# lcicek/Critic-VAE

Measured on AMD Instinct MI355X. Metric: VAE train-step images/sec on 64x64x3 frames, higher is better.
Workload: dtype f32

## Files before the change

### critic-vae_amd/csrc/api.hip

```cpp
#include "common.h"
#include "../../include/cvae.h"
#include <stdarg.h>
#include <stdio.h>
#include <stdlib.h>
#include <string.h>
#include <cmath>
#include <string>
#include <vector>

static thread_local char g_err[512] = "";
void cvae_set_error(const char* fmt, ...) {
    va_list ap;
    va_start(ap, fmt);
    vsnprintf(g_err, sizeof(g_err), fmt, ap);
    va_end(ap);
}

static constexpr int PROBE_IDS = 32, PROBE_CAP = 128;
struct ProbeSlot { hipEvent_t e0[PROBE_CAP], e1[PROBE_CAP]; int n = 0; bool made = false; };
struct ProbeState { uint32_t mask = 0; ProbeSlot slot[PROBE_IDS]; };
static thread_local ProbeSlot* g_probe_cur = nullptr;
void cvae_probe_begin(hipStream_t st) {
    ProbeSlot* p = g_probe_cur;
    if (p && p->n < PROBE_CAP) (void)hipEventRecord(p->e0[p->n], st);
}
void cvae_probe_end(hipStream_t st) {
    ProbeSlot* p = g_probe_cur;
    if (p && p->n < PROBE_CAP) { (void)hipEventRecord(p->e1[p->n], st); p->n++; }
}

int cvae_num_cus() {
    constexpr int NCACHE = 64;
    static std::atomic<int> cached[NCACHE];
    int dev = 0;
    hipError_t e = hipGetDevice(&dev);
    if (e != hipSuccess) { cvae_set_error("cvae_num_cus: hipGetDevice failed (%s); assuming 256 compute units", hipGetErrorString(e)); return 256; }
    const bool cacheable = dev >= 0 && dev < NCACHE;
    int n = cacheable ? cached[dev].load(std::memory_order_relaxed) : 0;
    if (n > 0) return n;
    e = hipDeviceGetAttribute(&n, hipDeviceAttributeMultiprocessorCount, dev);
    if (e != hipSuccess || n <= 0) {
        cvae_set_error("cvae_num_cus: compute-unit query failed on device %d (%s); assuming 256", dev, hipGetErrorString(e));
        return 256;
    }
    if (cacheable) cached[dev].store(n, std::memory_order_relaxed);
    return n;
}

int persistent_grid(int wgs_per_cu, int num_items) {
    static const int maxwg = [] { const char* e = getenv("CVAE_PERSIST_MAXWG"); const int n = e ? atoi(e) : 0; return n > 0 ? n : 0; }();
    int G = wgs_per_cu * cvae_num_cus();
    if (maxwg > 0 && G > maxwg) G = maxwg;
    G -= G % 8;
    if (G < 8) G = 8;
    return G < num_items ? G : num_items;
}
extern "C" int32_t cvae_conv_route(int32_t precision, int32_t width, int32_t layer, int32_t dgrad, int64_t batch) {
    if ((width != 64 && width != 128) || layer < 0 || layer > 3 || precision < 0 || precision > 3 || batch < 1 || batch > 0x7fffffffLL) return CVAE_EINVAL;
    if (layer == 0 && (precision != 1 || dgrad != 0)) return CVAE_EINVAL;
    return conv_route(precision, layer, width, dgrad != 0, batch).family;
}

struct ParamEntry { std::string name; int64_t offset, numel; };

struct WsLayout {
    int64_t y[4], a[4], coef[4], bnpart[4];
    int64_t zcat, h, o[4];
    int64_t dout4, d_o[4], d_h, d_zcat, d_a[4], d_y[4];
    int64_t wc[3];
    int64_t xp;
    int64_t wpack;
    int64_t ms, scratch_w, scratch, total;
};

struct cvae_handle_s {
    cvae_config cfg;
    std::vector<ParamEntry> params;
    int64_t param_total;
    int K;
    int enc_w[4], enc_b[4], enc_g[4], enc_be[4], fc_w, fc_b, dec_w[5], dec_b[5], di_w, di_b;
    hipStream_t side = nullptr;
    hipEvent_t ev_ready[8] = {}, ev_side = nullptr;
    bool streams_ready = false;
    const void* xp_ws = nullptr;
    int xp_B = 0;
    struct { int pass = 0, next = 0, B = 0; const void* ws = nullptr; const double* rec = nullptr; } sync;
    ProbeState probe;
};

struct ProbeArm {
    ProbeArm(cvae_handle_s* h, int kind, int layer) {
        const int id = kind * 9 + layer;
        g_probe_cur = (h->probe.mask >> id) & 1u ? &h->probe.slot[id] : nullptr;
    }
    ~ProbeArm() { g_probe_cur = nullptr; }
};

static int ensure_streams(cvae_handle_s* h) {
    if (h->streams_ready) return 0;
    int lo = 0, hi = 0;
    hipError_t e = hipDeviceGetStreamPriorityRange(&lo, &hi);
    if (e == hipSuccess) e = hipStreamCreateWithPriority(&h->side, hipStreamNonBlocking, lo);
    for (int i = 0; i < 8 && e == hipSuccess; ++i) e = hipEventCreateWithFlags(&h->ev_ready[i], hipEventDisableTiming);
    if (e == hipSuccess) e = hipEventCreateWithFlags(&h->ev_side, hipEventDisableTiming);
    if (e != hipSuccess) { cvae_set_error("side stream setup failed: %s", hipGetErrorString(e)); return (int)e; }
    h->streams_ready = true;
    return 0;
}

static int layer_h(const cvae_handle_s* h, int layer) { return kLayers[layer].h * (h->cfg.width / 64); }

static WsLayout carve(const cvae_handle_s* h, int B) {
    WsLayout w{};
    const int W = h->cfg.width;
    int64_t off = 0;
    auto take = [&](int64_t n) { int64_t o = off; off += align_up(n, 64); return o; };
    const bool b16 = h->cfg.precision == 1;
    auto act = [&](int64_t elems) { return take(b16 ? (elems + 1) / 2 : elems); };
    for (int l = 0; l < 4; ++l) {
        const int64_t H = layer_h(h, l), C = kLayers[l].cout;
        w.y[l] = act(B * H * H * C);
        w.a[l] = act(B * (H / 2) * (H / 2) * C);
        w.coef[l] = take(C * 4);
        w.bnpart[l] = take((int64_t)2 * bn_num_tiles(l, W, B) * C);
        w.d_y[l] = l == 0 ? -1 : act(B * H * H * C);
        w.d_a[l] = act(B * (H / 2) * (H / 2) * C);
    }
    w.zcat = take((int64_t)B * 33);
    w.d_zcat = take((int64_t)B * 33);
    w.h = act((int64_t)B * h->K);
    w.d_h = act((int64_t)B * h->K);
    for (int i = 0; i < 4; ++i) {
        const int64_t H = layer_h(h, 4 + i), C = kLayers[4 + i].cout;
        w.o[i] = act(B * H * H * C);
        w.d_o[i] = act(B * H * H * C);
    }
    w.dout4 = take(b16 ? 0 : (int64_t)B * 3 * W * W);
    for (int i = 0; i < 3; ++i) w.wc[i] = take(conv_up_wc_floats(5 + i));
    w.xp = take(b16 ? (int64_t)B * W * W * 2 : 0);
    w.wpack = take(h->cfg.precision != 0 ? conv_bf16_pack_floats(h->cfg.precision >= 2 ? 3 : 1) : 0);
    w.ms = take(msssim_ws_floats(W, B));
    int64_t sc = 0, scw = 0;
    auto mx = [&](int64_t v) { if (v > sc) sc = v; };
    for (int l = 1; l <= 4; ++l) { if (wgrad_ws_floats(l, W, B) > scw) scw = wgrad_ws_floats(l, W, B);
        if (h->cfg.precision == 1 && conv_bf16_supported(l, W) && wgrad_bf16_ws_floats(l, W, B) > scw) scw = wgrad_bf16_ws_floats(l, W, B);
        if (h->cfg.precision >= 2 && conv_bf16_supported(l, W) && wgrad_split_ws_floats(l, W, B) > scw) scw = wgrad_split_ws_floats(l, W, B);
        mx(conv_fwd_ws_floats(l, W, B)); mx(conv_dgrad_ws_floats(l, W, B)); }
    for (int l = 5; l <= 7; ++l) { if (conv_up_wgrad_ws_floats(l, W, B) > scw) scw = conv_up_wgrad_ws_floats(l, W, B); mx(conv_up_ws_floats(l, W, B)); }
    if (e1_wgrad_ws_floats(W, B) > scw) scw = e1_wgrad_ws_floats(W, B);
    w.scratch_w = take(scw);
    mx(scw + 36 * 128 * 64);
    mx(d4_bwd_ws_floats(W, B));
    for (int l = 0; l < 4; ++l) { mx(bn_bwd_ws_floats(l, W, B)); mx(bn_fwd_ws_floats(l, W)); }
    mx(fc_ws_floats(W, B));
    mx(colsum_ws_floats(0, 256));
    w.scratch = take(sc);
    w.total = off;
    return w;
}

static void add_param(cvae_handle_s* h, int* idx, const char* name, int64_t numel) {
    *idx = (int)h->params.size();
    h->params.push_back(ParamEntry{name, h->param_total, numel});
    h->param_total += align_up(numel, 64);
}

extern "C" {

const char* cvae_version(void) { return "critic-vae_amd 0.3 (gfx950; fp32 MFMA, bf16 MFMA with bf16 storage)"; }
const char* cvae_last_error(void) { return g_err; }

int cvae_create(const cvae_config* cfg, cvae_handle* out) {
    if (!cfg || !out) { cvae_set_error("cvae_create: null argument"); return CVAE_EINVAL; }
    if (cfg->width != 64 && cfg->width != 128) { cvae_set_error("cvae_create: width %d not supported (64 or 128)", cfg->width); return CVAE_EUNSUPPORTED; }
    if (cfg->precision < 0 || cfg->precision > 3) { cvae_set_error("cvae_create: precision %d not supported (0 = fp32, 1 = bf16 MFMA, 2 = fp32 emulated by 3-way bf16 splits)", cfg->precision); return CVAE_EUNSUPPORTED; }
    cvae_handle_s* h = new cvae_handle_s();
    h->cfg = *cfg;
    h->param_total = 0;
    h->K = 256 * (cfg->width / 16) * (cfg->width / 16);
    char nm[64];
    for (int l = 0; l < 4; ++l) {
        snprintf(nm, sizeof nm, "enc%d.w", l); add_param(h, &h->enc_w[l], nm, (int64_t)25 * kLayers[l].cin * kLayers[l].cout);
        snprintf(nm, sizeof nm, "enc%d.b", l); add_param(h, &h->enc_b[l], nm, kLayers[l].cout);
        snprintf(nm, sizeof nm, "enc%d.gamma", l); add_param(h, &h->enc_g[l], nm, kLayers[l].cout);
        snprintf(nm, sizeof nm, "enc%d.beta", l); add_param(h, &h->enc_be[l], nm, kLayers[l].cout);
    }
    add_param(h, &h->fc_w, "fc.w", (int64_t)h->K * 64);
    add_param(h, &h->fc_b, "fc.b", 64);
    for (int i = 0; i < 5; ++i) {
        snprintf(nm, sizeof nm, "dec%d.w", i); add_param(h, &h->dec_w[i], nm, (int64_t)25 * kLayers[4 + i].cin * kLayers[4 + i].cout);
        snprintf(nm, sizeof nm, "dec%d.b", i); add_param(h, &h->dec_b[i], nm, kLayers[4 + i].cout);
    }
    add_param(h, &h->di_w, "decin.w", (int64_t)33 * h->K);
    add_param(h, &h->di_b, "decin.b", h->K);
    *out = h;
    return CVAE_OK;
}

void cvae_destroy(cvae_handle h) {
    if (!h) return;
    if (h->streams_ready) {
        for (int i = 0; i < 8; ++i) (void)hipEventDestroy(h->ev_ready[i]);
        (void)hipEventDestroy(h->ev_side);
        (void)hipStreamDestroy(h->side);
    }
    delete h;
}

int64_t cvae_param_total(cvae_handle h) { return h->param_total; }
int32_t cvae_param_count(cvae_handle h) { return (int32_t)h->params.size(); }
const char* cvae_param_name(cvae_handle h, int32_t i) { return h->params[i].name.c_str(); }
int64_t cvae_param_offset(cvae_handle h, int32_t i) { return h->params[i].offset; }
int64_t cvae_param_numel(cvae_handle h, int32_t i) { return h->params[i].numel; }
int64_t cvae_workspace_bytes(cvae_handle h, int32_t batch) { return carve(h, batch).total * 4; }
int64_t cvae_bn_state_floats(cvae_handle) { return 2 * 480; }

int64_t cvae_ws_offset(cvae_handle h, int32_t batch, const char* name) {
    const WsLayout w = carve(h, batch);
    char nm[32];
    for (int l = 0; l < 4; ++l) {
        snprintf(nm, sizeof nm, "y%d", l); if (!strcmp(name, nm)) return w.y[l];
        snprintf(nm, sizeof nm, "a%d", l); if (!strcmp(name, nm)) return w.a[l];
        snprintf(nm, sizeof nm, "d_y%d", l); if (!strcmp(name, nm)) return w.d_y[l];
        snprintf(nm, sizeof nm, "d_a%d", l); if (!strcmp(name, nm)) return w.d_a[l];
        snprintf(nm, sizeof nm, "coef%d", l); if (!strcmp(name, nm)) return w.coef[l];
        snprintf(nm, sizeof nm, "o%d", l); if (!strcmp(name, nm)) return w.o[l];
        snprintf(nm, sizeof nm, "d_o%d", l); if (!strcmp(name, nm)) return w.d_o[l];
    }
    if (!strcmp(name, "zcat")) return w.zcat;
    if (!strcmp(name, "d_zcat")) return w.d_zcat;
    if (!strcmp(name, "h")) return w.h;
    if (!strcmp(name, "d_h")) return w.d_h;
    if (!strcmp(name, "dout4")) return w.dout4;
    if (!strcmp(name, "scratch")) return w.scratch;
    if (!strcmp(name, "ms")) return w.ms;
    if (!strcmp(name, "xp")) return h->cfg.precision == 1 ? w.xp : -1;
    return -1;
}

static const int kBnOff[4] = {0, 32, 96, 224};
static const int64_t kSyncOff[9] = {0, 97, 289, 673, 1441, 1452, 1964, 2220, 2348};
static const int64_t kSyncCnt[9] = {97, 192, 384, 768, 11, 512, 256, 128, 64};
static const int64_t kSyncCount = 96;
static_assert(2348 + 64 == CVAE_SYNC_DOUBLES, "sync record size");
int cvae_decode(cvae_handle h, int32_t B, const float* zcat, const float* params, float* recon, void* wsv, void* stream);
int cvae_backward_phases(cvae_handle h, int32_t B, const float* x, const float* pred, const float* eps, const float* params,
                         const float* logvar, const float* recon, const float* d_recon, const float* d_mu,
                         const float* d_logvar, void* wsv, float* grads, int32_t phase_mask, void* stream);

#define P_(idx) (params + h->params[(idx)].offset)
#define G_(idx) (grads + h->params[(idx)].offset)
#define RC(call) do { int rc_ = (call); if (rc_) return rc_; } while (0)

static bool use_bf16(cvae_handle h, int layer) {
    if (h->cfg.precision >= 2 && layer > 4) return false;
    return h->cfg.precision != 0 && conv_bf16_supported(layer, h->cfg.width);
}
static bool io_bf16(cvae_handle h) { return h->cfg.precision == 1; }
static bool use_bf16_wgrad(cvae_handle h, int layer) { return h->cfg.precision == 1 && conv_bf16_supported(layer, h->cfg.width); }
static bool use_split_wgrad(cvae_handle h, int layer) {
    if (h->cfg.precision < 2 || layer < 1 || layer > 4 || !conv_bf16_supported(layer, h->cfg.width)) return false;
    return conv_wgrad_split_supported(h->cfg.precision == 3 ? 6 : 9);
}
static int bf16_splits(cvae_handle h) { return h->cfg.precision >= 2 ? 3 : 1; }
static int bf16_mode(cvae_handle h) { return h->cfg.precision == 2 ? 3 : (h->cfg.precision == 3 ? 6 : 1); }
static int conv_wgrad(cvae_handle h, int layer, int B, const float* in, const float* dout, float* dw, float* dbias, float* ws, hipStream_t st) {
    const int W = h->cfg.width;
    if (use_bf16_wgrad(h, layer)) return launch_conv_wgrad_bf16(layer, W, B, in, dout, dw, dbias, ws, st);
    if (use_split_wgrad(h, layer)) return launch_conv_wgrad_split(layer, W, bf16_mode(h) == 6 ? 6 : 9, B, in, dout, dw, dbias, ws, st);
    return launch_conv_wgrad(layer, W, B, in, dout, dw, dbias, ws, st);
}
static int pack_bf16_weights(cvae_handle h, const float* params, float* ws, const WsLayout& w, hipStream_t st) {
    if (!use_bf16(h, 1)) return 0;
    const float* wl[4] = {P_(h->enc_w[1]), P_(h->enc_w[2]), P_(h->enc_w[3]), P_(h->dec_w[0])};
    return launch_pack_w_bf16(wl, ws + w.wpack, bf16_splits(h), st);
}

static int check(cvae_handle h, int32_t batch, const void* ws) {
    if (!h) { cvae_set_error("null handle"); return CVAE_EINVAL; }
    if (batch < 1 || batch > h->cfg.max_batch) { cvae_set_error("batch %d outside [1, %d]", batch, h->cfg.max_batch); return CVAE_EINVAL; }
    if (!ws) { cvae_set_error("null workspace"); return CVAE_ENOWS; }
    return 0;
}

struct FwdCtx {
    cvae_handle h; int B, W, train; const float* x; const float* params; float* bn_state; float* ws; void* wsv; WsLayout w; hipStream_t st;
    int tpp = 1;
    float* xp() const { return train && conv_route(1, 0, W, false, B).family == E1_PACKED_FRAME ? ws + w.xp : nullptr; }
    bool two_pass(int l) const { return l == 0 && h->cfg.precision == 1; }
    int conv(int l) {
        tpp = 1;
        if (two_pass(l)) {
            if (train) RC(launch_e1_fwd(W, B, x, P_(h->enc_w[0]), P_(h->enc_b[0]), nullptr, ws + w.bnpart[0], st, true, 1, nullptr, nullptr, xp()));
            h->xp_ws = xp() ? wsv : nullptr; h->xp_B = B;
            return 0;
        }
        if (l == 0) { ProbeArm pa(h, 0, 0); RC(launch_e1_fwd(W, B, x, P_(h->enc_w[0]), P_(h->enc_b[0]), ws + w.y[0], ws + w.bnpart[0], st)); }
        else if (use_bf16(h, l)) { ProbeArm pa(h, 0, l); RC(launch_conv_fwd_bf16(l, W, bf16_mode(h), B, ws + w.a[l - 1], ws + w.wpack, P_(h->enc_b[l]), ws + w.y[l], ws + w.bnpart[l], ws + w.scratch, st, &tpp)); }
        else { ProbeArm pa(h, 0, l); RC(launch_conv_fwd(l, W, B, ws + w.a[l - 1], P_(h->enc_w[l]), P_(h->enc_b[l]), ws + w.y[l], ws + w.bnpart[l], ws + w.scratch, st)); }
        return 0;
    }
    int stats(int l, double* sync) {
        if (sync) return launch_bn_fwd_record(l, W, B, ws + w.bnpart[l], ws + w.scratch, st, tpp, sync + kSyncOff[l], l == 0 ? sync + kSyncCount : nullptr);
        return launch_bn_fwd_finalize(l, W, B, ws + w.bnpart[l], P_(h->enc_g[l]), P_(h->enc_be[l]), bn_state + kBnOff[l],
                                      bn_state + 480 + kBnOff[l], ws + w.coef[l], ws + w.scratch, train, st, tpp);
    }
    int finish(int l, const double* sync) {
        return launch_bn_fwd_finish(l, W, sync + kSyncOff[l], sync + kSyncCount, P_(h->enc_g[l]), P_(h->enc_be[l]), bn_state + kBnOff[l],
                                    bn_state + 480 + kBnOff[l], ws + w.coef[l], st);
    }
    int apply(int l) {
        if (two_pass(l)) {
            ProbeArm pa(h, 0, 0);
            return launch_e1_fwd(W, B, x, P_(h->enc_w[0]), P_(h->enc_b[0]), ws + w.y[0], nullptr, st, true, 2, ws + w.coef[0], ws + w.a[0],
                                 xp());
        }
        return launch_bn_pool_act_fwd(l, W, B, ws + w.y[l], ws + w.coef[l], ws + w.a[l], st, io_bf16(h));
    }
};

int cvae_forward(cvae_handle h, int32_t B, const float* x, const float* pred, const float* eps, const float* params,
                 float* bn_state, float* mu, float* logvar, float* recon, void* wsv, int32_t train, void* stream) {
    RC(check(h, B, wsv));
    hipStream_t st = (hipStream_t)stream;
    float* ws = (float*)wsv;
    const WsLayout w = carve(h, B);
    const int W = h->cfg.width;
    RC(pack_bf16_weights(h, params, ws, w, st));
    FwdCtx f{h, B, W, train, x, params, bn_state, ws, wsv, w, st};
    for (int l = 0; l < 4; ++l) {
        RC(f.conv(l));
        RC(f.stats(l, nullptr));
        RC(f.apply(l));
    }
    RC(launch_fc_fwd(W, B, ws + w.a[3], P_(h->fc_w), P_(h->fc_b), eps, pred, mu, logvar, ws + w.zcat, ws + w.scratch, st, io_bf16(h)));
    if (!recon) return 0;
    return cvae_decode(h, B, nullptr, params, recon, wsv, stream);
}

int cvae_decode(cvae_handle h, int32_t B, const float* zcat, const float* params, float* recon, void* wsv, void* stream) {
    RC(check(h, B, wsv));
    hipStream_t st = (hipStream_t)stream;
    float* ws = (float*)wsv;
    const WsLayout w = carve(h, B);
    const int W = h->cfg.width;
    if (zcat) {
        hipError_t e = hipMemcpyAsync(ws + w.zcat, zcat, (size_t)B * 33 * sizeof(float), hipMemcpyDeviceToDevice, st);
        if (e != hipSuccess) { cvae_set_error("cvae_decode: copy failed: %s", hipGetErrorString(e)); return (int)e; }
        RC(pack_bf16_weights(h, params, ws, w, st));
    }
    RC(launch_decin_fwd(W, B, ws + w.zcat, P_(h->di_w), P_(h->di_b), ws + w.h, st, io_bf16(h)));
    {
        const float* wsrc[3] = {P_(h->dec_w[1]), P_(h->dec_w[2]), P_(h->dec_w[3])};
        float* wdst[3] = {ws + w.wc[0], ws + w.wc[1], ws + w.wc[2]};
        RC(launch_collapse_w3(wsrc, wdst, st));
    }
    if (use_bf16(h, 5)) {
        const float* wcs[3] = {ws + w.wc[0], ws + w.wc[1], ws + w.wc[2]};
        RC(launch_pack_up_bf16(wcs, ws + w.wpack, bf16_splits(h), st));
    }
    for (int i = 0; i < 4; ++i) {
        ProbeArm pa(h, 0, 4 + i);
        if (i == 0) {
// ... 980 lines not shown
```

### critic-vae_amd/csrc/common.h

```cpp
#pragma once
#include <hip/hip_runtime.h>
#include <stdint.h>
#include <stddef.h>
#include <atomic>

typedef float f32x16 __attribute__((ext_vector_type(16)));
typedef float f32x4 __attribute__((ext_vector_type(4)));
typedef __bf16 bf16x8 __attribute__((ext_vector_type(8)));

typedef __bf16 bf16x4 __attribute__((ext_vector_type(4)));

template <typename AT> struct Act;
template <> struct Act<float> {
    static constexpr bool BF16 = false;
    static __device__ __forceinline__ float ld(const float* p, size_t i) { return p[i]; }
    static __device__ __forceinline__ void st(float* p, size_t i, float v) { p[i] = v; }
    static __device__ __forceinline__ f32x4 ld4(const float* p, size_t i) { return *reinterpret_cast<const f32x4*>(p + i); }
    static __device__ __forceinline__ void st4(float* p, size_t i, f32x4 v) { *reinterpret_cast<f32x4*>(p + i) = v; }
    template <int V> using Vec = float __attribute__((ext_vector_type(V)));
    template <int V> static __device__ __forceinline__ Vec<V> ldv(const float* p, size_t i) {
        static_assert(V == 1 || V == 4, "fp32 storage: scalar or float4 accesses");
        return *reinterpret_cast<const Vec<V>*>(p + i);
    }
    template <int V> static __device__ __forceinline__ void stv(float* p, size_t i, Vec<V> v) {
        static_assert(V == 1 || V == 4, "fp32 storage: scalar or float4 accesses");
        *reinterpret_cast<Vec<V>*>(p + i) = v;
    }
};
template <> struct Act<__bf16> {
    static constexpr bool BF16 = true;
    static __device__ __forceinline__ float ld(const float* p, size_t i) { return (float)reinterpret_cast<const __bf16*>(p)[i]; }
    static __device__ __forceinline__ void st(float* p, size_t i, float v) { reinterpret_cast<__bf16*>(p)[i] = (__bf16)v; }
    static __device__ __forceinline__ f32x4 ld4(const float* p, size_t i) {
        const bf16x4 v = *reinterpret_cast<const bf16x4*>(reinterpret_cast<const __bf16*>(p) + i);
        return f32x4{(float)v[0], (float)v[1], (float)v[2], (float)v[3]};
    }
    static __device__ __forceinline__ void st4(float* p, size_t i, f32x4 v) {
        bf16x4 o;
        o[0] = (__bf16)v[0]; o[1] = (__bf16)v[1]; o[2] = (__bf16)v[2]; o[3] = (__bf16)v[3];
        *reinterpret_cast<bf16x4*>(reinterpret_cast<__bf16*>(p) + i) = o;
    }
    static __device__ __forceinline__ bf16x4 ld4raw(const float* p, size_t i) { return *reinterpret_cast<const bf16x4*>(reinterpret_cast<const __bf16*>(p) + i); }
    static __device__ __forceinline__ bf16x8 ld8(const float* p, size_t i) { return *reinterpret_cast<const bf16x8*>(reinterpret_cast<const __bf16*>(p) + i); }
    static __device__ __forceinline__ void st8(float* p, size_t i, bf16x8 v) { *reinterpret_cast<bf16x8*>(reinterpret_cast<__bf16*>(p) + i) = v; }
    template <int V> using Vec = __bf16 __attribute__((ext_vector_type(V)));
    template <int V> static __device__ __forceinline__ Vec<V> ldv(const float* p, size_t i) {
        static_assert(V == 8, "bf16 storage: 16-byte units of 8 elements");
        return ld8(p, i);
    }
    template <int V> static __device__ __forceinline__ void stv(float* p, size_t i, Vec<V> v) {
        static_assert(V == 8, "bf16 storage: 16-byte units of 8 elements");
        st8(p, i, v);
    }
};

typedef short short4v __attribute__((ext_vector_type(4)));
typedef short short8v __attribute__((ext_vector_type(8)));
__device__ __forceinline__ bf16x8 tr_frag(const __bf16* p0, const __bf16* p1) {
    const short4v lo = __builtin_amdgcn_ds_read_tr16_b64_v4i16((__attribute__((address_space(3))) short4v*)p0);
    const short4v hi = __builtin_amdgcn_ds_read_tr16_b64_v4i16((__attribute__((address_space(3))) short4v*)p1);
    const short8v v = __builtin_shufflevector(lo, hi, 0, 1, 2, 3, 4, 5, 6, 7);
    return __builtin_bit_cast(bf16x8, v);
}

#define CVAE_LATENT 32
#define CVAE_ZCAT 33

struct LayerDesc { int cin, cout, h, up; };
static constexpr LayerDesc kLayers[9] = {
    {3, 32, 64, 0}, {32, 64, 32, 0}, {64, 128, 16, 0}, {128, 256, 8, 0},
    {256, 128, 4, 0}, {128, 64, 8, 1}, {64, 32, 16, 1}, {32, 32, 32, 1}, {32, 3, 64, 1}};

struct TileGeom { int TW, TH, IMGS, PX_PER_IMG, TILES_PER_IMG; };
__host__ __device__ constexpr TileGeom tile_geom(int H) {
    const int TW = H < 32 ? H : 32;
    const int TH = (128 / TW) < H ? (128 / TW) : H;
    return TileGeom{TW, TH, 128 / (TW * TH), TW * TH, (H / TW) * (H / TH)};
}
template <int H>
struct Tile {
    static constexpr int TW = tile_geom(H).TW, TH = tile_geom(H).TH;
    static constexpr int IMGS = tile_geom(H).IMGS;
    static constexpr int HTW = TW + 4, HTH = TH + 4;
    static constexpr int HPI = HTW * HTH;
    static constexpr int HP = IMGS * HPI;
    static constexpr int PS = ((HP + 5) / 8) * 8 + 2;
    static constexpr int TILES_X = H / TW, TILES_Y = H / TH;
    static constexpr int TILES_PER_IMG = tile_geom(H).TILES_PER_IMG;
    static_assert(TW * TH * IMGS == 128, "tile must hold 128 pixels");
};

__host__ __device__ inline int cdiv(int a, int b) { return (a + b - 1) / b; }

__device__ __forceinline__ void vm_drained() { __builtin_amdgcn_s_waitcnt(0x0F70); }

__device__ __forceinline__ int xcd_tile(int x, int G) { return (G & 7) ? x : (x & 7) * (G >> 3) + (x >> 3); }
inline int64_t align_up(int64_t v, int64_t a) { return (v + a - 1) / a * a; }

__device__ __forceinline__ float wave_sum(float v) {
#pragma unroll
    for (int o = 32; o > 0; o >>= 1) v += __shfl_xor(v, o, 64);
    return v;
}
__device__ __forceinline__ double wave_sum_d(double v) {
#pragma unroll
    for (int o = 32; o > 0; o >>= 1) v += __shfl_xor(v, o, 64);
    return v;
}

__device__ __forceinline__ bool wg_arrive_last(unsigned* counter, unsigned total, unsigned* lds_word) {
    asm volatile("s_waitcnt vmcnt(0)" ::: "memory");
    __syncthreads();
    if (threadIdx.x == 0) {
        __builtin_amdgcn_fence(__ATOMIC_RELEASE, "agent");
        asm volatile("s_waitcnt vmcnt(0)" ::: "memory");
        const unsigned t = __hip_atomic_fetch_add(counter, 1u, __ATOMIC_RELAXED, __HIP_MEMORY_SCOPE_AGENT);
        const bool last = t == total - 1;
        if (last) {
            __hip_atomic_store(counter, 0u, __ATOMIC_RELAXED, __HIP_MEMORY_SCOPE_AGENT);
            __builtin_amdgcn_fence(__ATOMIC_ACQUIRE, "agent");
            asm volatile("s_waitcnt vmcnt(0)" ::: "memory");
        }
        *lds_word = last ? 1u : 0u;
    }
    __syncthreads();
    return *lds_word != 0u;
}

void cvae_probe_begin(hipStream_t st);
void cvae_probe_end(hipStream_t st);

void cvae_set_error(const char* fmt, ...);
#define CVAE_CHECK_LAUNCH()                                                        \
    do {                                                                           \
        hipError_t e_ = hipGetLastError();                                         \
        if (e_ != hipSuccess) {                                                    \
            cvae_set_error("%s:%d launch failed: %s", __FILE__, __LINE__,          \
                           hipGetErrorString(e_));                                 \
            return (int)e_;                                                        \
        }                                                                          \
    } while (0)

struct DeviceOnce { std::atomic<uint64_t> mask{0}; };
inline int cvae_grant_lds(DeviceOnce& once, const void* kernel, int bytes) {
    int dev = 0;
    hipError_t e = hipGetDevice(&dev);
    const uint64_t bit = 1ull << (dev & 63);
    if (e == hipSuccess && (once.mask.load(std::memory_order_acquire) & bit)) return 0;
    if (e == hipSuccess) e = hipFuncSetAttribute(kernel, hipFuncAttributeMaxDynamicSharedMemorySize, bytes);
    if (e != hipSuccess) { cvae_set_error("dynamic LDS opt-in (%d bytes) failed: %s", bytes, hipGetErrorString(e)); return (int)e; }
    once.mask.fetch_or(bit, std::memory_order_release);
    return 0;
}

int cvae_num_cus();
int persistent_grid(int wgs_per_cu, int num_items);

enum ConvFamily { CONV_PER_TILE = 0, CONV_PS = 1, CONV_BIG = 2, E1_PACKED_FRAME = 1 };
struct ConvRoute {
    ConvFamily family;
    int tilesPerPartial;
};
ConvRoute conv_route(int precision, int layer, int width, bool dgrad, int64_t B);

int launch_conv_fwd(int layer, int width, int B, const float* in, const float* w, const float* bias,
                    float* out, float* bnpart, float* ws, hipStream_t st);
int64_t conv_fwd_ws_floats(int layer, int width, int B);
int launch_conv_dgrad(int layer, int width, int B, const float* dout, const float* w,
                      const float* mask_src, float* din, float* ws, hipStream_t st);
int64_t conv_dgrad_ws_floats(int layer, int width, int B);
bool conv_bf16_supported(int layer, int width);
int64_t conv_bf16_pack_floats(int ns);
int launch_pack_w_bf16(const float* const w[4], float* packed, int ns, hipStream_t st);
int launch_conv_fwd_bf16(int layer, int width, int ns, int B, const float* in, const float* packed, const float* bias, float* out,
                         float* bnpart, float* ws, hipStream_t st, int* tilesPerPartial = nullptr);
int launch_conv_dgrad_bf16(int layer, int width, int ns, int B, const float* dout, const float* packed, float* din, float* ws, hipStream_t st);
int launch_pack_up_bf16(const float* const wc[3], float* packed, int ns, hipStream_t st);
int launch_conv_up_fwd_bf16(int layer, int width, int ns, int B, const float* in, const float* packed, const float* bias, float* out, hipStream_t st);
int launch_conv_up_dgrad_bf16(int layer, int width, int ns, int B, const float* dout, const float* packed, const float* aux, float* din, hipStream_t st);
int64_t wgrad_bf16_ws_floats(int layer, int width, int B);
int launch_conv_wgrad_bf16(int layer, int width, int B, const float* in, const float* dout, float* dw, float* dbias, float* ws, hipStream_t st);
bool conv_wgrad_split_supported(int products);
int64_t wgrad_split_ws_floats(int layer, int width, int B);
int launch_conv_wgrad_split(int layer, int width, int products, int B, const float* in, const float* dout, float* dw, float* dbias,
                            float* ws, hipStream_t st);
int launch_splitk_bias_relu(const float* slab, const float* bias, float* out, int64_t slice, int KS, int C, hipStream_t st, bool out_bf16 = false);
int64_t wgrad_ws_floats(int layer, int width, int B);
int launch_conv_wgrad(int layer, int width, int B, const float* in, const float* dout, float* dw,
                      float* dbias, float* ws, hipStream_t st);
int launch_reduce_slabs(const float* slab, float* dst, int64_t n, int S, int64_t stride, hipStream_t st,
                        float* mid = nullptr, bool out_bf16 = false);
int launch_colsum(const float* src, int64_t rows, int C, float* dst, float* ws, hipStream_t st);
int64_t colsum_ws_floats(int64_t rows, int C);
static constexpr int CS_BLOCKS = 128;
__device__ __forceinline__ void colsum_stage1_block(const float* __restrict__ src, int64_t rows, int C, float* __restrict__ part,
                                                    int blk, int nblk, float* red) {
    const int c = threadIdx.x % C, rl = threadIdx.x / C, RL = 256 / C;
    const int64_t per = (rows + nblk - 1) / nblk;
    const int64_t r0 = blk * per;
    int64_t r1 = r0 + per; if (r1 > rows) r1 = rows;
    float acc = 0.f;
    for (int64_t r = r0 + rl; r < r1; r += RL) acc += src[r * C + c];
    red[threadIdx.x] = acc;
    __syncthreads();
    if (rl == 0) {
        for (int k = 1; k < RL; ++k) acc += red[k * C + c];
        part[(size_t)blk * C + c] = acc;
    }
}
int64_t col_reduce_ws_floats(int W);
int launch_col_reduce_partial(const float* in, int R, int W, int64_t stride, float* ws, hipStream_t st,
                              const float** rows_out, int* R_out, int64_t* stride_out);
int launch_col_reduce(const float* in, int R, int W, int64_t stride, float* out, float* ws, hipStream_t st, int skip_col0 = -1);
int launch_e1_fwd(int width, int B, const float* x, const float* w, const float* bias, float* y,
                  float* bnpart, hipStream_t st, bool bf16 = false, int pass = 0, const float* coef = nullptr, float* a1 = nullptr,
                  float* xp = nullptr);
int launch_e1_wgrad(int width, int B, const float* x, const float* dy, float* dw, float* dbias, float* ws,
                    hipStream_t st, bool bf16 = false, const float* const* fuse = nullptr,
                    const float* xp = nullptr);
const float* bn_bwd_bcoef(int layer, int width, int B, const float* ws);
int64_t e1_wgrad_ws_floats(int width, int B);
int launch_d4_fwd(int width, int B, const float* in, const float* w, const float* bias, float* recon,
                  hipStream_t st, bool bf16io = false);
int64_t d4_bwd_ws_floats(int width, int B);
int launch_d4_bwd(int width, int B, const float* o3, const float* d_recon, const float* recon,
                  const float* w, float* dout, float* d_o3, float* dw, float* db, float* ws,
                  hipStream_t st, bool bf16io = false);
int64_t conv_up_wc_floats(int layer);
int launch_collapse_w(int layer, const float* w, float* wc, hipStream_t st);
int launch_collapse_w3(const float* const w[3], float* const wc[3], hipStream_t st);
int64_t conv_up_ws_floats(int layer, int width, int B);
int launch_conv_up_fwd(int layer, int width, int B, const float* in, const float* wc, const float* bias,
                       float* out, float* ws, hipStream_t st);
int launch_conv_up_dgrad(int layer, int width, int B, const float* dout, const float* wc, const float* aux,
                         float* din, float* ws, hipStream_t st);
int64_t conv_up_wgrad_ws_floats(int layer, int width, int B);
int launch_conv_up_wgrad(int layer, int width, int B, const float* in, const float* dout, float* dw,
                         float* dbias, float* ws, hipStream_t st, bool bf16 = false);
int launch_up_wgrad_bf16_main(int layer, int width, int B, const float* in, const float* dout, float* slab, int Smax, int* S_out, hipStream_t st,
                              int* plan = nullptr);
int conv_wgrad_bf16_plan(int layer, int width, int B, int plan[3]);
int conv_up_wgrad_bf16_plan(int layer, int width, int B, int plan[3]);
int bn_num_tiles(int layer, int width, int B);
int launch_bn_fwd_finalize(int layer, int width, int B, const float* bnpart, const float* gamma,
                           const float* beta, float* run_mean, float* run_var, float* coef,
                           float* ws, int train, hipStream_t st, int tilesPerPartial = 1);
int launch_bn_fwd_record(int layer, int width, int B, const float* bnpart, float* ws, hipStream_t st, int tilesPerPartial,
                         double* rec, double* count);
int launch_bn_fwd_finish(int layer, int width, const double* rec, const double* count, const float* gamma, const float* beta,
                         float* run_mean, float* run_var, float* coef, hipStream_t st);
int64_t bn_fwd_ws_floats(int layer, int width);
int launch_bn_pool_act_fwd(int layer, int width, int B, const float* y, const float* coef, float* a,
                           hipStream_t st, bool bf16io = false);
int64_t bn_bwd_ws_floats(int layer, int width, int B);
int launch_bn_pool_act_bwd(int layer, int width, int B, const float* y, const float* a,
                           const float* da, const float* coef, const float* gamma, float* dy,
                           float* dgamma, float* dbeta, float* dbias, float* ws, hipStream_t st, bool bf16io = false,
                           int stage = 0, double* rec = nullptr, const double* count = nullptr);
struct LatentPlan {
    int fc_fwd_gemm;
    int di_imgs, di_blocks;
    int db_bgemm, db_gemm;
    int df_imgs, fb_bgemm, fb_dflat, fb_colsum;
    int fb_split;
};
LatentPlan latent_plan(int width, int B, int num_cus);
int64_t fc_ws_floats(int width, int B);
int launch_fc_fwd(int width, int B, const float* flat, const float* wfc, const float* bfc,
                  const float* eps, const float* pred, float* mu, float* logvar, float* zcat,
                  float* ws, hipStream_t st, bool bf16io = false);
int launch_decin_fwd(int width, int B, const float* zcat, const float* wd, const float* bd, float* h,
                     hipStream_t st, bool bf16io = false);
int launch_decin_bwd(int width, int B, const float* zcat, const float* dh, const float* wd, float* dwd,
                     float* dbd, float* dzcat, float* ws, hipStream_t st, bool bf16io = false);
int launch_fc_bwd(int width, int B, const float* flat, const float* wfc, const float* dzcat,
                  const float* eps, const float* logvar, const float* dmu_loss,
                  const float* dlv_loss, float* dwfc, float* dbfc, float* dflat, float* ws,
                  hipStream_t st, bool bf16io = false);
struct LossObjective { float w_ms, w_mse, kw; int used; };
constexpr int MSSSIM_SLAB_DOUBLES = 32 * 11;
int launch_objective_pixels(int width, int B, const float* recon, const float* x, const float* const* F, const float* coef,
                            float* dx, const float* mu, const float* logvar, float* d_mu, float* d_logvar,
                            LossObjective obj, double* slab, unsigned* ticket, float* scalars, hipStream_t st);
int64_t msssim_ws_floats(int width, int B);
int launch_msssim(int width, int B, const float* img1, const float* img2, const float* mu,
                  const float* logvar, float* ws, float* scalars, float* d_img1, float* d_mu,
                  float* d_logvar, hipStream_t st,
                  int stage = 0, double* rec = nullptr, const double* images = nullptr,
                  const LossObjective* obj = nullptr);
void msssim_score_slots(int width, int B, int64_t part[5], int64_t* scratch);
int launch_msssim_finish_rec(int width, const double* rec, const double* images, float* scalars, float* coef, hipStream_t st);
int64_t score_state_bytes();
int launch_score_init(void* state, hipStream_t st);
int launch_score(int width, int B, const float* x, const float* mu, const float* logvar, const float* recon, float* ms,
                 float* per_image, void* state, hipStream_t st);
int launch_score_finish(int width, void* state, float* scalars, hipStream_t st);
namespace critic_layout {
constexpr int CW1 = 0, CB1 = 216, CW2 = 224, CB2 = 800, CW3 = 808, CB3 = 1384, CW4 = 1392, CB4 = 2544,
              CW5 = 2560, CB5 = 10752, CF1W = 10784, CF1B = 11808, CF2W = 11840, CF2B = 11872;
constexpr int CRITIC_PARAMS = 11873;
}
int critic_param_count();
int launch_critic_fwd(int width, int B, const float* x, const float* critic_params, float* pred, hipStream_t st);
int launch_preprocess_u8(int width, int B, const uint8_t* u8, float* x, hipStream_t st);
int critic_train_floats();
int64_t critic_grad_scratch_bytes(int B);
int launch_critic_grad(int width, int B, const float* x, const float* target, const uint8_t* keep, float scale, int loss_kind,
                       const float* critic_params, float* grads, float* pred, float* loss_scalars, uint8_t* decisions,
                       void* scratch, hipStream_t st);
int64_t critic_score_state_bytes();
int64_t critic_score_scratch_bytes(int B);
int launch_critic_score_init(void* state, hipStream_t st);
int launch_critic_score(int B, const uint8_t* frames, const float* targets, int64_t n, const int64_t* idx, const float* critic_params,
                        float* rows, void* state, hipStream_t st);
int launch_critic_collect(int B, const float* x, const float* critic_params, float* pred, float* const e[5], hipStream_t st);
int launch_critic_saliency(int B, const float* x, const float* critic_params, int steps, float* pred, float* grad, float* map,
                           float* max_values, uint8_t* decisions, hipStream_t st);
int launch_critic_occlusion(int B, const float* x, const float* critic_params, int patch, float fill_r, float fill_g, float fill_b,
                            float* pred, float* drop, float* map, float* max_values, hipStream_t st);
int launch_curate_select(int n_traj, const int64_t* off, int64_t n_frames, const float* preds, int collect,
                         int64_t total_images, int64_t* running, int64_t* counts, int64_t* first, int64_t* span,
                         int64_t* sel, hipStream_t st);
int launch_gather_frames_u8(int width, const uint8_t* src, const float* src_pred, int64_t n_src, const int64_t* sel,
                            int64_t max_count, const int64_t* span, uint8_t* dst, float* dst_pred, int64_t capacity,
                            hipStream_t st);
int launch_preprocess_u8_gather(int width, int B, const uint8_t* frames, const float* preds, int64_t n, const int64_t* idx,
                                float* x, float* pred, hipStream_t st);
int launch_curate_select_recon(int n_traj, const int64_t* off, int64_t n_frames, const float* preds, int collect,
                               int64_t total_images, int64_t* running, int64_t* counts, int64_t* first, int64_t* sel_first,
                               int64_t* span, int64_t* ent_frame, int32_t* ent_kind, int64_t* ent_sel, int64_t* sel,
                               hipStream_t st);
int launch_recon_zcat(int n_entries, const int64_t* ent_sel, const int32_t* ent_kind, const float* mu, const float* sel_pred,
                      int64_t n_sel, float* zcat, hipStream_t st);
int launch_inject_zcat(int n_images, int n_rewards, const float* mu, const float* rewards, float* zcat, hipStream_t st);
int launch_gather_f32(int width, int B, const float* frames, const float* preds, int64_t n, const int64_t* idx, float* x,
                      float* pred, hipStream_t st);
int launch_preprocess_u8_gather_aug(int width, int B, const uint8_t* frames, const float* preds, int64_t n, const int64_t* idx,
                                    const struct cvae_augment& aug, float* x, float* pred, int32_t* applied, hipStream_t st);
int launch_gather_f32_aug(int width, int B, const float* frames, const float* preds, int64_t n, const int64_t* idx,
                          const struct cvae_augment& aug, float* x, float* pred, int32_t* applied, hipStream_t st);
int launch_diff_grey(int width, int B, const float* a, const float* b, float* diff, hipStream_t st);
int64_t crf_scratch_bytes(int width, int B);
int launch_dense_crf(int width, int B, const uint8_t* frames, const float* prob1, const struct cvae_crf_params& p,
                     uint8_t* labels, float* q1, void* scratch, hipStream_t st);
int launch_diff_normalize(int width, int B, const float* diff, double mean_max, double factor, int thr, const uint8_t* gt,
                          uint8_t* u8, uint8_t* mask, int64_t* counts, int64_t* hist, hipStream_t st);
int launch_mask_counts(int width, int B, const uint8_t* mask, const uint8_t* gt, int64_t* counts, hipStream_t st);
int launch_compose_frames(int width, int B, int n_panels, const struct cvae_panel* panels, int ih, int clamp, const uint8_t* overlay,
                          const uint8_t* atlas, int n_labels, int lh, int lw, const int32_t* label_idx, int lx, int ly,
                          uint8_t* out, hipStream_t st);
int launch_grads_bf16(const float* src_f32, void* bf16_buf, float* dst_f32, int64_t n, hipStream_t st);
int launch_adam(float* p, const float* g, float* m, float* v, int64_t n, int step, float lr, float b1,
                float b2, float eps, float gscale, hipStream_t st);
int64_t guard_state_bytes();
int launch_guard_init(void* state, int64_t applied, int64_t skipped, hipStream_t st);
int launch_grad_stats(const float* g, int64_t n, float gscale, float max_norm, int skip_nonfinite, float lr, float b1, float b2,
                      void* state, hipStream_t st);
int launch_adam_guarded(float* p, const float* g, float* m, float* v, int64_t n, float eps, const void* state, hipStream_t st);
struct cvae_opt_args;
int launch_adam_opt(float* p, const float* g, float* m, float* v, int64_t n, int step, float lr, float b1, float b2, float eps,
                    float gscale, const cvae_opt_args* opt, float* ema, const float* aux, float* aux_ema, int32_t n_aux, hipStream_t st);
int launch_adam_guarded_opt(float* p, const float* g, float* m, float* v, int64_t n, float eps, const void* state,
                            const cvae_opt_args* opt, float* ema, const float* aux, float* aux_ema, int32_t n_aux, hipStream_t st);
struct cvae_tensor_stat;
int launch_trace_push(void* ring, int64_t capacity, int64_t step, float lr, const float* scalars, int n_scalars,
                      const void* guard_state, hipStream_t st);
int launch_tensor_stats(const float* p, const float* g, const float* m, const float* v, int64_t n, int32_t n_tensors,
                        const int64_t* begin, const int64_t* end, int64_t step, float lr, float b1, float b2, float eps, float gscale,
                        const void* guard_state, cvae_tensor_stat* out, void* scratch, hipStream_t st);
int64_t tensor_stats_scratch_bytes(int32_t n_tensors, const int64_t* begin, const int64_t* end);
int tensor_stats_plan(int32_t n_tensors, const int64_t* begin, const int64_t* end, int32_t* chunk, int32_t* items, int32_t* grid);
int launch_zero(float* p, int64_t n, hipStream_t st);
struct PadGaps { int64_t off[32]; int len[32]; int n; };
int launch_zero_gaps(float* grads, const PadGaps& gaps, hipStream_t st);
struct Scale3 { const float* g; const float* src[3]; float* dst[3]; int64_t n[3]; };
int launch_scale3(const Scale3& a, hipStream_t st);
```

### critic-vae_amd/csrc/conv_mfma.hip

```cpp
#include "common.h"
#include "conv_epilogue.h"


struct ConvRouteRow { int precision, layer, width; bool dgrad; ConvFamily family; int tilesPerPartial; };
static constexpr ConvRouteRow kConvRoutes[] = {
    {0, 1, 64, false, CONV_PS, 1}, {0, 2, 64, false, CONV_PS, 1}, {0, 3, 64, false, CONV_PS, 1},
    {0, 2, 64, true, CONV_PS, 1}, {0, 3, 64, true, CONV_PS, 1},
    {0, 1, 128, false, CONV_PS, 1}, {0, 2, 128, false, CONV_PS, 1}, {0, 2, 128, true, CONV_PS, 1},
    {1, 1, 64, false, CONV_BIG, 8}, {1, 2, 64, false, CONV_BIG, 4}, {1, 3, 64, false, CONV_BIG, 4},
    {1, 1, 64, true, CONV_BIG, 1}, {1, 2, 64, true, CONV_BIG, 1}, {1, 3, 64, true, CONV_BIG, 1},
    {1, 1, 128, false, CONV_BIG, 8}, {1, 2, 128, false, CONV_BIG, 4}, {1, 3, 128, false, CONV_BIG, 4},
    {1, 1, 128, true, CONV_BIG, 1}, {1, 2, 128, true, CONV_BIG, 1}, {1, 3, 128, true, CONV_BIG, 1},
    {1, 4, 128, false, CONV_PS, 1},
    {1, 0, 64, false, E1_PACKED_FRAME, 1}, {1, 0, 128, false, E1_PACKED_FRAME, 1},
};

ConvRoute conv_route(int precision, int layer, int width, bool dgrad, int64_t B) {
    static const bool per_tile_only = [] { const char* e = getenv("CVAE_CONV_PER_TILE"); return e && e[0] == '1'; }();
    const ConvRoute per_tile{CONV_PER_TILE, 1};
    for (const ConvRouteRow& r : kConvRoutes) {
        if (r.precision != precision || r.layer != layer || r.width != width || r.dgrad != dgrad) continue;
        if (layer == 0) {
            if (B * width * width * 8 + (2 * width + 2) * 8 >= (1ll << 31)) return per_tile;
            return {r.family, r.tilesPerPartial};
        }
        if (per_tile_only) return per_tile;
        const int64_t h = kLayers[layer].h * width / 64, c = kLayers[layer].cin > kLayers[layer].cout ? kLayers[layer].cin : kLayers[layer].cout;
        if (B * h * h * c * (precision == 1 ? 2 : 4) >= (1ll << 31)) return per_tile;
        return {r.family, r.tilesPerPartial};
    }
    return per_tile;
}


struct ConvArgs {
    const float* in;
    const float* w;
    const float* bias;
    const float* aux;
    float* out;
    float* bnpart;
    int B;
    int64_t sliceFloats;
};

template <int NT> struct KChunk { static constexpr int KC = NT == 32 ? 32 : 16, KCP = KC + 1; };


template <int KCH, int NCH, int H, bool DGRAD, int NT, int EPI, int KSPLIT>
__global__ __launch_bounds__(256) void conv5x5_mfma_kernel(ConvArgs a) {
    using T = Tile<H>;
    constexpr int NB = NT / 32;
    constexpr int KC = KChunk<NT>::KC, KCP = KChunk<NT>::KCP, QPP = KC / 4;
    constexpr int IN_FLOATS = KC * T::PS;
    constexpr int W_FLOATS = DGRAD ? 5 * NT * KCP : 5 * KC * NT;
    constexpr int EPI_FLOATS = (EPI == EPI_POOLSUM_MASK) ? 128 * (NT + 1) : 4 * 32 * 36;
    constexpr int SMEM = (IN_FLOATS + W_FLOATS) > EPI_FLOATS ? (IN_FLOATS + W_FLOATS) : EPI_FLOATS;
    __shared__ __attribute__((aligned(16))) float smem[SMEM];
    float* lds_in = smem;
    float* lds_w = smem + IN_FLOATS;

    const int tid = threadIdx.x, lane = tid & 63, wave = tid >> 6;
    const int li = lane & 31, lh = lane >> 5;
    const int mt = xcd_tile(blockIdx.x, gridDim.x), n0 = blockIdx.y * NT;
    const int tileInImg = mt % T::TILES_PER_IMG;
    const int img0 = (mt / T::TILES_PER_IMG) * T::IMGS;
    const int ty0 = (tileInImg / T::TILES_X) * T::TH, tx0 = (tileInImg % T::TILES_X) * T::TW;

    const int m = wave * 32 + li;
    const int pimg = m / (T::TH * T::TW), prem = m % (T::TH * T::TW);
    const int aBase = lh * T::PS + pimg * T::HPI + (prem / T::TW) * T::HTW + (prem % T::TW);
    const int bBase = DGRAD ? (li * KCP + lh) : (lh * NT + li);

    f32x16 acc[NB];
#pragma unroll
    for (int nb = 0; nb < NB; ++nb)
#pragma unroll
        for (int v = 0; v < 16; ++v) acc[nb][v] = 0.f;

    constexpr int WQ = 5 * KC * NT / 4;
    constexpr int WPT = (WQ + 255) / 256;
    f32x4 wreg[WPT];

    auto load_w = [&](int st) {
        const int cc = st / 5, r = st % 5;
#pragma unroll
        for (int i = 0; i < WPT; ++i) {
            const int q = tid + i * 256;
            if (WQ % 256 == 0 || q < WQ) {
                const float* src;
                if (!DGRAD) {
                    const int row = q / (NT / 4), c4 = q % (NT / 4);
                    const int s = row / KC, kc = row % KC;
                    src = a.w + (size_t)((r * 5 + s) * KCH + cc * KC + kc) * NCH + n0 + c4 * 4;
                } else {
                    const int c4 = q % QPP, rown = q / QPP;
                    const int n = rown % NT, s = rown / NT;
                    src = a.w + (size_t)((24 - (r * 5 + s)) * NCH + n0 + n) * KCH + cc * KC + c4 * 4;
                }
                wreg[i] = *reinterpret_cast<const f32x4*>(src);
            }
        }
    };
    auto store_w = [&]() {
#pragma unroll
        for (int i = 0; i < WPT; ++i) {
            const int q = tid + i * 256;
            if (WQ % 256 == 0 || q < WQ) {
                if (!DGRAD) {
                    *reinterpret_cast<f32x4*>(lds_w + q * 4) = wreg[i];
                } else {
                    const int c4 = q % QPP, rown = q / QPP;
                    float* d = lds_w + rown * KCP + c4 * 4;
                    d[0] = wreg[i].x; d[1] = wreg[i].y; d[2] = wreg[i].z; d[3] = wreg[i].w;
                }
            }
        }
    };
    constexpr int NQ = T::HP * (KC / 4), IPT = (NQ + 255) / 256;
    f32x4 ireg[IPT];
    auto load_input = [&](int cc) {
#pragma unroll
        for (int i = 0; i < IPT; ++i) {
            const int q = tid + i * 256;
            const int c4 = q % QPP, hp = q / QPP;
            const int img = hp / T::HPI, rem = hp - img * T::HPI;
            const int hy = rem / T::HTW, hx = rem - hy * T::HTW;
            const int gy = ty0 + hy - 2, gx = tx0 + hx - 2, ib = img0 + img;
            f32x4 v = {0.f, 0.f, 0.f, 0.f};
            if ((NQ % 256 == 0 || q < NQ) && (unsigned)gy < (unsigned)H && (unsigned)gx < (unsigned)H && ib < a.B)
                v = *reinterpret_cast<const f32x4*>(a.in + ((size_t)(ib * H + gy) * H + gx) * KCH + cc * KC + c4 * 4);
            ireg[i] = v;
        }
    };
    auto store_input = [&]() {
#pragma unroll
        for (int i = 0; i < IPT; ++i) {
            const int q = tid + i * 256;
            if (NQ % 256 == 0 || q < NQ) {
                float* d = lds_in + ((q % QPP) * 4) * T::PS + (q / QPP);
                d[0] = ireg[i].x; d[T::PS] = ireg[i].y; d[2 * T::PS] = ireg[i].z; d[3 * T::PS] = ireg[i].w;
            }
        }
    };

    static_assert((KCH / KC) % KSPLIT == 0, "split-K must divide the channel chunks");
    constexpr int NST = (KCH / KC) / KSPLIT * 5;
    const int st0 = blockIdx.z * NST, st1 = st0 + NST;
    [[maybe_unused]] float biasv[NB];
    if constexpr (KSPLIT == 1 && (EPI == EPI_BIAS_BNSTAT || EPI == EPI_BIAS_RELU)) load_bias<NT, EPI>(biasv, a.bias, n0);
    load_w(st0);
    load_input(st0 / 5);
    for (int st = st0; st < st1; ++st) {
        const int r = st % 5;
        __syncthreads();
        if (r == 0) store_input();
        store_w();
        if (r == 0 && st + 5 < st1) load_input(st / 5 + 1);
        if (st + 1 < st1) load_w(st + 1);
        __syncthreads();
        const float* ap = lds_in + aBase + r * T::HTW;
        __builtin_amdgcn_iglp_opt(0);
#pragma unroll
        for (int s = 0; s < 5; ++s) {
#pragma unroll
            for (int j = 0; j < KC / 2; ++j) {
                const float av = ap[(2 * j) * T::PS + s];
#pragma unroll
                for (int nb = 0; nb < NB; ++nb) {
                    const float bv = DGRAD ? lds_w[bBase + (s * NT + nb * 32) * KCP + 2 * j]
                                           : lds_w[bBase + (s * KC + 2 * j) * NT + nb * 32];
                    acc[nb] = __builtin_amdgcn_mfma_f32_32x32x2f32(av, bv, acc[nb], 0, 0, 0);
                }
            }
        }
    }
    vm_drained();

    if (KSPLIT > 1) {
        epilogue_store<H, NT, NCH, EPI_PLAIN>(acc, a.out + (size_t)blockIdx.z * a.sliceFloats, nullptr, smem, a.B,
                                              mt, n0, img0, ty0, tx0);
    } else if (EPI == EPI_BIAS_BNSTAT || EPI == EPI_BIAS_RELU || EPI == EPI_PLAIN) {
        apply_bias<NT, EPI>(acc, biasv);
        __builtin_amdgcn_sched_barrier(0);
        epilogue_store<H, NT, NCH, EPI>(acc, a.out, a.bnpart, smem, a.B, mt, n0, img0, ty0, tx0);
    } else {
        __syncthreads();
        float* lo = smem;
#pragma unroll
        for (int nb = 0; nb < NB; ++nb)
#pragma unroll
            for (int v = 0; v < 16; ++v) {
                const int mm = wave * 32 + (v & 3) + 8 * (v >> 2) + 4 * lh;
                lo[mm * (NT + 1) + nb * 32 + li] = acc[nb][v];
            }
        __syncthreads();
        constexpr int PTW = T::TW / 2, PTH = T::TH / 2, HO = H / 2;
        for (int q = tid; q < 32 * NT; q += 256) {
            const int c = q % NT, pp = q / NT;
            const int im = pp / (PTW * PTH), rem = pp % (PTW * PTH);
            const int py = rem / PTW, px = rem % PTW, ib = img0 + im;
            if (ib >= a.B) continue;
            const int m00 = im * T::TH * T::TW + (2 * py) * T::TW + 2 * px;
            const float sum = (lo[m00 * (NT + 1) + c] + lo[(m00 + 1) * (NT + 1) + c]) +
                              (lo[(m00 + T::TW) * (NT + 1) + c] + lo[(m00 + T::TW + 1) * (NT + 1) + c]);
            const size_t o = ((size_t)(ib * HO + ty0 / 2 + py) * HO + tx0 / 2 + px) * NCH + n0 + c;
            a.out[o] = a.aux[o] > 0.f ? sum : 0.f;
        }
    }
}

template <int KCH, int NCH, int H, bool DGRAD, int NT, int EPI, int KSPLIT = 1>
static int run(const ConvArgs& a, hipStream_t st) {
    using T = Tile<H>;
    static_assert(KCH % KChunk<NT>::KC == 0 && NCH % NT == 0, "channel tiling");
    dim3 grid(cdiv(a.B, T::IMGS) * T::TILES_PER_IMG, NCH / NT, KSPLIT);
    cvae_probe_begin(st);
    hipLaunchKernelGGL((conv5x5_mfma_kernel<KCH, NCH, H, DGRAD, NT, EPI, KSPLIT>), grid, dim3(256), 0, st, a);
    cvae_probe_end(st);
    CVAE_CHECK_LAUNCH();
    return 0;
}

template <int KCH, int NCH, bool DGRAD, int NT, int KSPLIT>
__global__ __launch_bounds__(256) void conv4x4_row_kernel(ConvArgs a) {
    constexpr int NB = NT / 32;
    constexpr int KC = KChunk<NT>::KC, KCP = KChunk<NT>::KCP, QPP = KC / 4;
    constexpr int PXS = 33, PS = 16 * PXS + 2;
    constexpr int IN_FLOATS = KC * PS;
    constexpr int W_FLOATS = DGRAD ? 5 * NT * KCP : 5 * KC * NT;
    __shared__ __attribute__((aligned(16))) float smem[IN_FLOATS + W_FLOATS];
    float* lds_in = smem;
    float* lds_w = smem + IN_FLOATS;
    static_assert(IN_FLOATS % 4 == 0, "weight slab stays 16-byte aligned");
    const int tid = threadIdx.x, lane = tid & 63, wave = tid >> 6, li = lane & 31, lh = lane >> 5;
    const int ya = (blockIdx.x & 1) * 2, img0 = (blockIdx.x >> 1) * 32, n0 = blockIdx.y * NT;
    const int r0 = ya == 0 ? 1 : 0, r1 = ya == 0 ? 4 : 3;
    const int aBase = lh * PS + li;
    const int bBase = DGRAD ? (li * KCP + lh) : (lh * NT + li);

    f32x16 acc[2][NB];
#pragma unroll
    for (int t = 0; t < 2; ++t)
#pragma unroll
        for (int nb = 0; nb < NB; ++nb)
#pragma unroll
            for (int v = 0; v < 16; ++v) acc[t][nb][v] = 0.f;

    constexpr int WQ = 5 * KC * NT / 4, WPT = (WQ + 255) / 256;
    f32x4 wreg[WPT];
    auto load_w = [&](int cc, int r) {
#pragma unroll
        for (int i = 0; i < WPT; ++i) {
            const int q = tid + i * 256;
            if (WQ % 256 == 0 || q < WQ) {
                const float* src;
                if (!DGRAD) {
                    const int row = q / (NT / 4), c4 = q % (NT / 4);
                    const int s = row / KC, kc = row % KC;
                    src = a.w + (size_t)((r * 5 + s) * KCH + cc * KC + kc) * NCH + n0 + c4 * 4;
                } else {
                    const int c4 = q % QPP, rown = q / QPP;
                    const int n = rown % NT, s = rown / NT;
                    src = a.w + (size_t)((24 - (r * 5 + s)) * NCH + n0 + n) * KCH + cc * KC + c4 * 4;
                }
                wreg[i] = *reinterpret_cast<const f32x4*>(src);
            }
        }
    };
    auto store_w = [&]() {
#pragma unroll
        for (int i = 0; i < WPT; ++i) {
            const int q = tid + i * 256;
            if (WQ % 256 == 0 || q < WQ) {
                if (!DGRAD) {
                    *reinterpret_cast<f32x4*>(lds_w + q * 4) = wreg[i];
                } else {
                    const int c4 = q % QPP, rown = q / QPP;
                    float* d = lds_w + rown * KCP + c4 * 4;
                    d[0] = wreg[i].x; d[1] = wreg[i].y; d[2] = wreg[i].z; d[3] = wreg[i].w;
                }
            }
        }
    };
    constexpr int NQ = 512 * QPP, IPT = NQ / 256;
    f32x4 ireg[IPT];
    auto load_input = [&](int cc) {
#pragma unroll
        for (int i = 0; i < IPT; ++i) {
            const int q = tid + i * 256, c4 = q % QPP, hp = q / QPP, ib = img0 + (hp >> 4);
            f32x4 v = {0.f, 0.f, 0.f, 0.f};
            if (ib < a.B) v = *reinterpret_cast<const f32x4*>(a.in + ((size_t)ib * 16 + (hp & 15)) * KCH + cc * KC + c4 * 4);
            ireg[i] = v;
        }
    };
    auto store_input = [&]() {
#pragma unroll
        for (int i = 0; i < IPT; ++i) {
            const int q = tid + i * 256, c4 = q % QPP, hp = q / QPP;
            float* d = lds_in + (c4 * 4) * PS + (hp & 15) * PXS + (hp >> 4);
            d[0] = ireg[i].x; d[PS] = ireg[i].y; d[2 * PS] = ireg[i].z; d[3 * PS] = ireg[i].w;
        }
    };

    static_assert((KCH / KC) % KSPLIT == 0, "split-K must divide the channel chunks");
    constexpr int CPS = (KCH / KC) / KSPLIT;
    const int c0 = blockIdx.z * CPS, c1 = c0 + CPS;
    load_w(c0, r0);
    load_input(c0);
    for (int cc = c0; cc < c1; ++cc)
        for (int r = r0; r <= r1; ++r) {
            __syncthreads();
            if (r == r0) store_input();
            store_w();
            if (r == r0 && cc + 1 < c1) load_input(cc + 1);
            if (r < r1) load_w(cc, r + 1);
            else if (cc + 1 < c1) load_w(cc + 1, r0);
            __syncthreads();
#pragma unroll
            for (int t = 0; t < 2; ++t) {
                const int yi = ya + t + r - 2;
                if ((unsigned)yi > 3u) continue;
                const int xc = wave ^ t;
                const int s0 = xc < 2 ? 2 - xc : 0, s1 = xc > 1 ? 5 - xc : 4;
                const float* ap = lds_in + aBase + (yi * 4 + xc - 2) * PXS;
                for (int s = s0; s <= s1; ++s) {
                    const float* as = ap + s * PXS;
                    const float* bs = lds_w + bBase + (DGRAD ? s * NT * KCP : s * KC * NT);
#pragma unroll
                    for (int j = 0; j < KC / 2; ++j) {
                        const float av = as[(2 * j) * PS];
#pragma unroll
                        for (int nb = 0; nb < NB; ++nb) {
                            const float bv = DGRAD ? bs[nb * 32 * KCP + 2 * j] : bs[(2 * j) * NT + nb * 32];
                            acc[t][nb] = __builtin_amdgcn_mfma_f32_32x32x2f32(av, bv, acc[t][nb], 0, 0, 0);
                        }
                    }
                }
            }
        }
    vm_drained();
    float* out = a.out + (size_t)blockIdx.z * a.sliceFloats;
#pragma unroll
    for (int t = 0; t < 2; ++t)
#pragma unroll
        for (int nb = 0; nb < NB; ++nb)
#pragma unroll
            for (int v = 0; v < 16; ++v) {
                const int ib = img0 + (v & 3) + 8 * (v >> 2) + 4 * lh;
                if (ib < a.B) out[((size_t)ib * 16 + (ya + t) * 4 + (wave ^ t)) * NCH + n0 + nb * 32 + li] = acc[t][nb][v];
            }
}

template <int KCH, int NCH, bool DGRAD, int NT, int KSPLIT>
static int run4x4(const ConvArgs& a, hipStream_t st) {
    static_assert(KCH % KChunk<NT>::KC == 0 && NCH % NT == 0, "channel tiling");
    cvae_probe_begin(st);
    hipLaunchKernelGGL((conv4x4_row_kernel<KCH, NCH, DGRAD, NT, KSPLIT>), dim3(cdiv(a.B, 32) * 2, NCH / NT, KSPLIT), dim3(256), 0, st, a);
    cvae_probe_end(st);
    CVAE_CHECK_LAUNCH();
    return 0;
}

template <typename AT>
__global__ __launch_bounds__(256) void splitk_bias_relu_kernel(const float* __restrict__ slab, const float* __restrict__ bias,
                                                               float* __restrict__ out, int64_t n4, int64_t slice, int KS, int C) {
    const int64_t i = (int64_t)blockIdx.x * 256 + threadIdx.x;
    if (i >= n4) return;
    float4 acc = *reinterpret_cast<const float4*>(bias + (i * 4) % C);
    for (int z = 0; z < KS; ++z) {
        const float4 v = *reinterpret_cast<const float4*>(slab + (size_t)z * slice + i * 4);
        acc.x += v.x; acc.y += v.y; acc.z += v.z; acc.w += v.w;
    }
    acc.x = fmaxf(acc.x, 0.f); acc.y = fmaxf(acc.y, 0.f); acc.z = fmaxf(acc.z, 0.f); acc.w = fmaxf(acc.w, 0.f);
    Act<AT>::st4(out, (size_t)i * 4, f32x4{acc.x, acc.y, acc.z, acc.w});
}

int launch_splitk_bias_relu(const float* slab, const float* bias, float* out, int64_t slice, int KS, int C, hipStream_t st, bool out_bf16) {
    if (out_bf16) hipLaunchKernelGGL(splitk_bias_relu_kernel<__bf16>, dim3((unsigned)((slice / 4 + 255) / 256)), dim3(256), 0, st, slab, bias, out,
                                     slice / 4, slice, KS, C);
    else hipLaunchKernelGGL(splitk_bias_relu_kernel<float>, dim3((unsigned)((slice / 4 + 255) / 256)), dim3(256), 0, st, slab, bias, out,
                       slice / 4, slice, KS, C);
    CVAE_CHECK_LAUNCH();
    return 0;
}

static constexpr int D0_KSPLIT = 8;
int64_t conv_fwd_ws_floats(int layer, int width, int B) {
    if (layer != 4 || width != 64) return 0;
    const int64_t h = kLayers[4].h * (width / 64);
    return (int64_t)D0_KSPLIT * B * h * h * kLayers[4].cout;
}

int launch_conv_mfma_ps(int layer, int width, bool dgrad, int B, const float* in, const float* w, const float* bias, float* out, float* bnpart, hipStream_t st);

int launch_conv_fwd(int layer, int width, int B, const float* in, const float* w, const float* bias,
                    float* out, float* bnpart, float* ws, hipStream_t st) {
    if (conv_route(0, layer, width, false, B).family == CONV_PS) return launch_conv_mfma_ps(layer, width, false, B, in, w, bias, out, bnpart, st);
    ConvArgs a{in, w, bias, nullptr, out, bnpart, B, 0};
    if (width == 64) {
        switch (layer) {
            case 1: return run<32, 64, 32, false, 64, EPI_BIAS_BNSTAT>(a, st);
            case 2: return run<64, 128, 16, false, 64, EPI_BIAS_BNSTAT>(a, st);
            case 3: return run<128, 256, 8, false, 32, EPI_BIAS_BNSTAT>(a, st);
            case 4: {
                const int64_t slice = (int64_t)B * 4 * 4 * 128;
                a.out = ws; a.sliceFloats = slice;
                int rc = run4x4<256, 128, false, 64, D0_KSPLIT>(a, st);
                if (rc) return rc;
                hipLaunchKernelGGL(splitk_bias_relu_kernel<float>, dim3((unsigned)((slice / 4 + 255) / 256)), dim3(256), 0, st,
                                   ws, bias, out, slice / 4, slice, D0_KSPLIT, 128);
                CVAE_CHECK_LAUNCH();
                return 0;
            }
        }
    }
    if (width == 128) {
        switch (layer) {
            case 1: return run<32, 64, 64, false, 64, EPI_BIAS_BNSTAT>(a, st);
            case 2: return run<64, 128, 32, false, 64, EPI_BIAS_BNSTAT>(a, st);
            case 3: return run<128, 256, 16, false, 64, EPI_BIAS_BNSTAT>(a, st);
            case 4: return run<256, 128, 8, false, 64, EPI_BIAS_RELU>(a, st);
        }
    }
    cvae_set_error("conv_fwd: unsupported layer %d at width %d", layer, width);
    return -2;
}

static constexpr int D0_DGRAD_KSPLIT = 4;
int64_t conv_dgrad_ws_floats(int layer, int width, int B) {
    if (layer != 4 || width != 64) return 0;
    return (int64_t)D0_DGRAD_KSPLIT * B * 16 * kLayers[4].cin;
}

int launch_conv_dgrad(int layer, int width, int B, const float* dout, const float* w,
                      const float* mask_src, float* din, float* ws, hipStream_t st) {
    if (!mask_src && conv_route(0, layer, width, true, B).family == CONV_PS) return launch_conv_mfma_ps(layer, width, true, B, dout, w, nullptr, din, nullptr, st);
    ConvArgs a{dout, w, nullptr, mask_src, din, nullptr, B, 0};
    if (width == 64 && layer == 4 && ws != nullptr) {
        const int64_t slice = (int64_t)B * 16 * 256;
        a.out = ws; a.sliceFloats = slice;
        int rc = run4x4<128, 256, true, 64, D0_DGRAD_KSPLIT>(a, st);
        if (rc) return rc;
        return launch_reduce_slabs(ws, din, slice, D0_DGRAD_KSPLIT, slice, st, nullptr);
    }
    if (width == 64) {
        switch (layer) {
            case 1: return run<64, 32, 32, true, 32, EPI_PLAIN>(a, st);
            case 2: return run<128, 64, 16, true, 64, EPI_PLAIN>(a, st);
            case 3: return run<256, 128, 8, true, 32, EPI_PLAIN>(a, st);
            case 4: return run<128, 256, 4, true, 32, EPI_PLAIN>(a, st);
        }
    }
    if (width == 128) {
        switch (layer) {
            case 1: return run<64, 32, 64, true, 32, EPI_PLAIN>(a, st);
            case 2: return run<128, 64, 32, true, 64, EPI_PLAIN>(a, st);
            case 3: return run<256, 128, 16, true, 64, EPI_PLAIN>(a, st);
            case 4: return run<128, 256, 8, true, 64, EPI_PLAIN>(a, st);
        }
    }
    cvae_set_error("conv_dgrad: unsupported layer %d at width %d", layer, width);
    return -2;
}
```

### critic-vae_amd/csrc/conv_up.hip

```cpp
#include "common.h"

static constexpr int KC = 16, KCP = 17;

template <int HS>
struct UpTile {
    static constexpr int TW = HS < 32 ? HS : 32;
    static constexpr int TH = (128 / TW) < HS ? (128 / TW) : HS;
    static constexpr int IMGS = 128 / (TW * TH);
    static constexpr int HTW = TW + 2, HTH = TH + 2, HPI = HTW * HTH, HP = IMGS * HPI;
    static constexpr int PS = ((HP + 5) / 8) * 8 + 2;
    static constexpr int TILES_X = HS / TW, TILES_Y = HS / TH, TILES_PER_IMG = TILES_X * TILES_Y;
};

__device__ __forceinline__ int phase_lo(int ph, int a) { return ph == 0 ? (a == 0 ? 0 : a == 1 ? 2 : 4) : (a == 0 ? 0 : a == 1 ? 1 : 3); }
__device__ __forceinline__ int phase_hi(int ph, int a) { return ph == 0 ? (a == 0 ? 1 : a == 1 ? 3 : 4) : (a == 0 ? 0 : a == 1 ? 2 : 4); }
__device__ __forceinline__ int phase_of(int ph, int r) { return ph == 0 ? (r >> 1) : ((r + 1) >> 1); }

struct CollapseJobs { const float* w[3]; float* wc[3]; int n[3]; };
__global__ __launch_bounds__(256) void collapse_w_kernel(CollapseJobs jobs) {
    const float* __restrict__ w = jobs.w[blockIdx.z];
    float* __restrict__ wc = jobs.wc[blockIdx.z];
    const int n = jobs.n[blockIdx.z];
    const int i = blockIdx.x * 256 + threadIdx.x;
    if (i >= n) return;
    const int t = blockIdx.y, p = t / 9, a = (t % 9) / 3, b = t % 3, py = p >> 1, px = p & 1;
    float acc = 0.f;
    for (int r = phase_lo(py, a); r <= phase_hi(py, a); ++r)
        for (int s = phase_lo(px, b); s <= phase_hi(px, b); ++s) acc += w[(size_t)(r * 5 + s) * n + i];
    wc[(size_t)t * n + i] = acc;
}

__global__ __launch_bounds__(256) void expand_dw_kernel(const float* __restrict__ rows, int R, int64_t stride,
                                                        float* __restrict__ dw, int n, float* __restrict__ dbias,
                                                        int cout) {
    const int i = blockIdx.x * 256 + threadIdx.x;
    if (dbias != nullptr && blockIdx.x == 0 && blockIdx.y == 0 && (int)threadIdx.x < cout) {
        float b = 0.f;
        for (int q = 0; q < R; ++q) b += rows[(size_t)q * stride + (size_t)36 * n + threadIdx.x];
        dbias[threadIdx.x] = b;
    }
    if (i >= n) return;
    const int r = blockIdx.y / 5, s = blockIdx.y % 5;
    float acc = 0.f;
#pragma unroll
    for (int p = 0; p < 4; ++p) {
        const float* src = rows + (size_t)(p * 9 + phase_of(p >> 1, r) * 3 + phase_of(p & 1, s)) * n + i;
        float a = 0.f;
        for (int q = 0; q < R; ++q) a += src[(size_t)q * stride];
        acc += a;
    }
    dw[(size_t)blockIdx.y * n + i] = acc;
}

struct UpArgs {
    const float* in;
    const float* wc;
    const float* bias;
    const float* aux;
    float* out;
    int B;
    int64_t sliceFloats;
};

template <int CIN, int COUT, int HS, int KSPLIT>
__global__ __launch_bounds__(256) void conv_up_fwd_kernel(UpArgs a) {
    using T = UpTile<HS>;
    constexpr int NT = 32, H = 2 * HS;
    constexpr int IN_FLOATS = KC * T::PS, W_FLOATS = 12 * KC * NT;
    __shared__ __attribute__((aligned(16))) float smem[IN_FLOATS + W_FLOATS];
    float* lds_in = smem;
    float* lds_w = smem + IN_FLOATS;
    const int tid = threadIdx.x, lane = tid & 63, wave = tid >> 6, li = lane & 31, lh = lane >> 5;
    const int mt = xcd_tile(blockIdx.x, gridDim.x), n0 = blockIdx.y * NT;
    const int tileInImg = mt % T::TILES_PER_IMG, img0 = (mt / T::TILES_PER_IMG) * T::IMGS;
    const int ty0 = (tileInImg / T::TILES_X) * T::TH, tx0 = (tileInImg % T::TILES_X) * T::TW;
    const int m = wave * 32 + li;
    const int pimg = m / (T::TH * T::TW), prem = m % (T::TH * T::TW);
    const int aBase = lh * T::PS + pimg * T::HPI + (prem / T::TW) * T::HTW + (prem % T::TW);
    const int bBase = lh * NT + li;

    f32x16 acc[4];
#pragma unroll
    for (int p = 0; p < 4; ++p)
#pragma unroll
        for (int v = 0; v < 16; ++v) acc[p][v] = 0.f;

    constexpr int WQ = 12 * KC * NT / 4, WPT = WQ / 256;
    f32x4 wreg[WPT];
    auto load_w = [&](int st) {
        const int cc = st / 3, ar = st % 3;
#pragma unroll
        for (int i = 0; i < WPT; ++i) {
            const int q = tid + i * 256;
            const int row = q / (NT / 4), c4 = q % (NT / 4);
            const int pb = row / KC, kc = row % KC, p = pb / 3, b = pb % 3;
            wreg[i] = *reinterpret_cast<const f32x4*>(
                a.wc + ((size_t)(p * 9 + ar * 3 + b) * CIN + cc * KC + kc) * COUT + n0 + c4 * 4);
        }
    };
    auto store_w = [&]() {
#pragma unroll
        for (int i = 0; i < WPT; ++i) *reinterpret_cast<f32x4*>(lds_w + (tid + i * 256) * 4) = wreg[i];
    };
    constexpr int NQ = T::HP * (KC / 4), IPT = (NQ + 255) / 256;
    f32x4 ireg[IPT];
    auto load_input = [&](int cc) {
#pragma unroll
        for (int i = 0; i < IPT; ++i) {
            const int q = tid + i * 256;
            const int c4 = q & 3, hp = q >> 2;
            const int img = hp / T::HPI, rem = hp - img * T::HPI;
            const int gy = ty0 + rem / T::HTW - 1, gx = tx0 + rem % T::HTW - 1, ib = img0 + img;
            f32x4 v = {0.f, 0.f, 0.f, 0.f};
            if ((NQ % 256 == 0 || q < NQ) && (unsigned)gy < (unsigned)HS && (unsigned)gx < (unsigned)HS && ib < a.B)
                v = *reinterpret_cast<const f32x4*>(a.in + ((size_t)(ib * HS + gy) * HS + gx) * CIN + cc * KC + c4 * 4);
            ireg[i] = v;
        }
    };
    auto store_input = [&]() {
#pragma unroll
        for (int i = 0; i < IPT; ++i) {
            const int q = tid + i * 256;
            if (NQ % 256 == 0 || q < NQ) {
                float* d = lds_in + ((q & 3) * 4) * T::PS + (q >> 2);
                d[0] = ireg[i].x; d[T::PS] = ireg[i].y; d[2 * T::PS] = ireg[i].z; d[3 * T::PS] = ireg[i].w;
            }
        }
    };

    static_assert((CIN / KC) % KSPLIT == 0, "split-K must divide the channel chunks");
    constexpr int NST = (CIN / KC) / KSPLIT * 3;
    const int st0 = blockIdx.z * NST, st1 = st0 + NST;
    const float bv = KSPLIT > 1 ? 0.f : a.bias[n0 + li];
    load_w(st0);
    load_input(st0 / 3);
    for (int st = st0; st < st1; ++st) {
        const int ar = st % 3;
        __syncthreads();
        if (ar == 0) store_input();
        store_w();
        if (ar == 0 && st + 3 < st1) load_input(st / 3 + 1);
        if (st + 1 < st1) load_w(st + 1);
        __syncthreads();
        const float* ap = lds_in + aBase + ar * T::HTW;
        __builtin_amdgcn_iglp_opt(0);
#pragma unroll
        for (int b = 0; b < 3; ++b)
#pragma unroll
            for (int j = 0; j < KC / 2; ++j) {
                const float av = ap[(2 * j) * T::PS + b];
#pragma unroll
                for (int p = 0; p < 4; ++p)
                    acc[p] = __builtin_amdgcn_mfma_f32_32x32x2f32(av, lds_w[bBase + ((p * 3 + b) * KC + 2 * j) * NT], acc[p], 0, 0, 0);
            }
    }
    vm_drained();
    float* out = KSPLIT > 1 ? a.out + (size_t)blockIdx.z * a.sliceFloats : a.out;
#pragma unroll
    for (int p = 0; p < 4; ++p)
#pragma unroll
        for (int v = 0; v < 16; ++v) {
            const int mm = wave * 32 + (v & 3) + 8 * (v >> 2) + 4 * lh;
            const int im = mm / (T::TH * T::TW), rem = mm % (T::TH * T::TW);
            const int oy = 2 * (ty0 + rem / T::TW) + (p >> 1), ox = 2 * (tx0 + rem % T::TW) + (p & 1), ib = img0 + im;
            float x = acc[p][v] + bv;
            if (KSPLIT == 1) x = fmaxf(x, 0.f);
            if (ib < a.B) out[((size_t)(ib * H + oy) * H + ox) * COUT + n0 + li] = x;
        }
}

template <int CIN, int COUT, int HS, int NT, int KSPLIT>
__global__ __launch_bounds__(256) void conv_up_dgrad_kernel(UpArgs a) {
    using T = UpTile<HS>;
    constexpr int NB = NT / 32, H = 2 * HS;
    constexpr int IN_FLOATS = KC * T::PS, W_FLOATS = 9 * NT * KCP;
    __shared__ __attribute__((aligned(16))) float smem[IN_FLOATS + W_FLOATS];
    float* lds_in = smem;
    float* lds_w = smem + IN_FLOATS;
    const int tid = threadIdx.x, lane = tid & 63, wave = tid >> 6, li = lane & 31, lh = lane >> 5;
    const int mt = xcd_tile(blockIdx.x, gridDim.x), n0 = blockIdx.y * NT;
    const int tileInImg = mt % T::TILES_PER_IMG, img0 = (mt / T::TILES_PER_IMG) * T::IMGS;
    const int ty0 = (tileInImg / T::TILES_X) * T::TH, tx0 = (tileInImg % T::TILES_X) * T::TW;
    const int m = wave * 32 + li;
    const int pimg = m / (T::TH * T::TW), prem = m % (T::TH * T::TW);
    const int aBase = lh * T::PS + pimg * T::HPI + (prem / T::TW + 2) * T::HTW + (prem % T::TW) + 2;
    const int bBase = li * KCP + lh;

    f32x16 acc[NB];
#pragma unroll
    for (int nb = 0; nb < NB; ++nb)
#pragma unroll
        for (int v = 0; v < 16; ++v) acc[nb][v] = 0.f;

    constexpr int WQ = 9 * NT * KC / 4, WPT = (WQ + 255) / 256;
    f32x4 wreg[WPT];
    auto load_w = [&](int st) {
        const int cc = st / 4, p = st % 4;
#pragma unroll
        for (int i = 0; i < WPT; ++i) {
            const int q = tid + i * 256;
            if (WQ % 256 == 0 || q < WQ) {
                const int c4 = q & 3, rown = q >> 2, n = rown % NT, t = rown / NT;
                wreg[i] = *reinterpret_cast<const f32x4*>(
                    a.wc + ((size_t)(p * 9 + t) * CIN + n0 + n) * COUT + cc * KC + c4 * 4);
            }
        }
    };
    auto store_w = [&]() {
#pragma unroll
        for (int i = 0; i < WPT; ++i) {
            const int q = tid + i * 256;
            if (WQ % 256 == 0 || q < WQ) {
                float* d = lds_w + (q >> 2) * KCP + (q & 3) * 4;
                d[0] = wreg[i].x; d[1] = wreg[i].y; d[2] = wreg[i].z; d[3] = wreg[i].w;
            }
        }
    };
    constexpr int NQ = T::HP * (KC / 4), IPT = (NQ + 255) / 256;
    f32x4 ireg[IPT];
    auto load_input = [&](int st) {
        const int cc = st / 4, py = (st % 4) >> 1, px = st & 1;
#pragma unroll
        for (int i = 0; i < IPT; ++i) {
            const int q = tid + i * 256;
            const int c4 = q & 3, hp = q >> 2;
            const int img = hp / T::HPI, rem = hp - img * T::HPI;
            const int yy = ty0 + rem / T::HTW - 1, xx = tx0 + rem % T::HTW - 1, ib = img0 + img;
            f32x4 v = {0.f, 0.f, 0.f, 0.f};
            if ((NQ % 256 == 0 || q < NQ) && (unsigned)yy < (unsigned)HS && (unsigned)xx < (unsigned)HS && ib < a.B)
                v = *reinterpret_cast<const f32x4*>(
                    a.in + ((size_t)(ib * H + 2 * yy + py) * H + 2 * xx + px) * COUT + cc * KC + c4 * 4);
            ireg[i] = v;
        }
    };
    auto store_input = [&]() {
#pragma unroll
        for (int i = 0; i < IPT; ++i) {
            const int q = tid + i * 256;
            if (NQ % 256 == 0 || q < NQ) {
                float* d = lds_in + ((q & 3) * 4) * T::PS + (q >> 2);
                d[0] = ireg[i].x; d[T::PS] = ireg[i].y; d[2 * T::PS] = ireg[i].z; d[3 * T::PS] = ireg[i].w;
            }
        }
    };

    static_assert((COUT / KC) % KSPLIT == 0, "split-K must divide the channel chunks");
    constexpr int NST = (COUT / KC) / KSPLIT * 4;
    const int st0 = blockIdx.z * NST, st1 = st0 + NST;
    load_w(st0);
    load_input(st0);
    for (int st = st0; st < st1; ++st) {
        __syncthreads();
        store_input();
        store_w();
        if (st + 1 < st1) { load_input(st + 1); load_w(st + 1); }
        __syncthreads();
        __builtin_amdgcn_iglp_opt(0);
#pragma unroll
        for (int t = 0; t < 9; ++t)
#pragma unroll
            for (int j = 0; j < KC / 2; ++j) {
                const float av = lds_in[aBase + (2 * j) * T::PS - (t / 3) * T::HTW - (t % 3)];
#pragma unroll
                for (int nb = 0; nb < NB; ++nb)
                    acc[nb] = __builtin_amdgcn_mfma_f32_32x32x2f32(av, lds_w[bBase + (t * NT + nb * 32) * KCP + 2 * j], acc[nb], 0, 0, 0);
            }
    }
    vm_drained();
    float* out = KSPLIT > 1 ? a.out + (size_t)blockIdx.z * a.sliceFloats : a.out;
    size_t o[NB][16];
    float mk[NB][16];
#pragma unroll
    for (int nb = 0; nb < NB; ++nb)
#pragma unroll
        for (int v = 0; v < 16; ++v) {
            const int mm = wave * 32 + (v & 3) + 8 * (v >> 2) + 4 * lh;
            const int im = mm / (T::TH * T::TW), rem = mm % (T::TH * T::TW), ib = img0 + im;
            o[nb][v] = ((size_t)(ib * HS + ty0 + rem / T::TW) * HS + tx0 + rem % T::TW) * CIN + n0 + nb * 32 + li;
            if (KSPLIT == 1) mk[nb][v] = a.aux[ib < a.B ? o[nb][v] : 0];
        }
#pragma unroll
    for (int nb = 0; nb < NB; ++nb)
#pragma unroll
        for (int v = 0; v < 16; ++v) {
            const int mm = wave * 32 + (v & 3) + 8 * (v >> 2) + 4 * lh;
            if (img0 + mm / (T::TH * T::TW) >= a.B) continue;
            float x = acc[nb][v];
            if (KSPLIT == 1) x = mk[nb][v] > 0.f ? x : 0.f;
            out[o[nb][v]] = x;
        }
}

__global__ __launch_bounds__(256) void up_finish_relu_kernel(const float* __restrict__ slab, const float* __restrict__ bias,
                                                             float* __restrict__ out, int64_t n4, int64_t slice, int KS, int C) {
    const int64_t i = (int64_t)blockIdx.x * 256 + threadIdx.x;
    if (i >= n4) return;
    float4 acc = *reinterpret_cast<const float4*>(bias + (i * 4) % C);
    for (int z = 0; z < KS; ++z) {
        const float4 v = *reinterpret_cast<const float4*>(slab + (size_t)z * slice + i * 4);
        acc.x += v.x; acc.y += v.y; acc.z += v.z; acc.w += v.w;
    }
    acc.x = fmaxf(acc.x, 0.f); acc.y = fmaxf(acc.y, 0.f); acc.z = fmaxf(acc.z, 0.f); acc.w = fmaxf(acc.w, 0.f);
    *reinterpret_cast<float4*>(out + i * 4) = acc;
}
__global__ __launch_bounds__(256) void up_finish_mask_kernel(const float* __restrict__ slab, const float* __restrict__ aux,
                                                             float* __restrict__ out, int64_t n4, int64_t slice, int KS) {
    const int64_t i = (int64_t)blockIdx.x * 256 + threadIdx.x;
    if (i >= n4) return;
    float4 acc = make_float4(0.f, 0.f, 0.f, 0.f);
    for (int z = 0; z < KS; ++z) {
        const float4 v = *reinterpret_cast<const float4*>(slab + (size_t)z * slice + i * 4);
        acc.x += v.x; acc.y += v.y; acc.z += v.z; acc.w += v.w;
    }
    const float4 m = *reinterpret_cast<const float4*>(aux + i * 4);
    acc.x = m.x > 0.f ? acc.x : 0.f; acc.y = m.y > 0.f ? acc.y : 0.f;
    acc.z = m.z > 0.f ? acc.z : 0.f; acc.w = m.w > 0.f ? acc.w : 0.f;
    *reinterpret_cast<float4*>(out + i * 4) = acc;
}

template <int HS>
struct UpTile64 {
    static constexpr int TW = HS < 16 ? HS : 16;
    static constexpr int TH = (64 / TW) < HS ? (64 / TW) : HS;
    static constexpr int IMGS = 64 / (TW * TH);
    static constexpr int HTW = TW + 2, HTH = TH + 2, HPI = HTW * HTH, HP = IMGS * HPI;
    static constexpr int TILES_X = HS / TW, TILES_Y = HS / TH, TILES_PER_IMG = TILES_X * TILES_Y;
};

struct UpWgradArgs {
    const float* in;
    const float* dout;
    float* slab;
    int B, numTiles, tilesPerSplit;
};

template <int CIN, int COUT, int HS>
__global__ __launch_bounds__(256, 2) void conv_up_wgrad_kernel(UpWgradArgs a) {
    using T = UpTile64<HS>;
    constexpr int H = 2 * HS, CS = 32, IN_FLOATS = T::HP * CS;
    __shared__ __attribute__((aligned(16))) float smem[IN_FLOATS + 4 * 64 * 32];
    float* lds_in = smem;
    float* lds_d = smem + IN_FLOATS;
    const int tid = threadIdx.x, lane = tid & 63, wave = tid >> 6, li = lane & 31, lh = lane >> 5;
    const int split = blockIdx.x, ci0 = blockIdx.y * 32, n0 = blockIdx.z * 32;
    f32x16 acc[9];
    float bsum = 0.f;
#pragma unroll
    for (int t = 0; t < 9; ++t)
#pragma unroll
        for (int v = 0; v < 16; ++v) acc[t][v] = 0.f;
    const int t0 = split * a.tilesPerSplit;
    int t1 = t0 + a.tilesPerSplit; if (t1 > a.numTiles) t1 = a.numTiles;
    constexpr int IQ = (T::HP * 8 + 255) / 256;
    f32x4 rin[IQ], rdo[8];
    auto fetch = [&](int mt) {
        const int tileInImg = mt % T::TILES_PER_IMG, img0 = (mt / T::TILES_PER_IMG) * T::IMGS;
        const int ty0 = (tileInImg / T::TILES_X) * T::TH, tx0 = (tileInImg % T::TILES_X) * T::TW;
#pragma unroll
        for (int i = 0; i < IQ; ++i) {
            const int q = tid + i * 256;
            const int c4 = q & 7, hp = q >> 3;
            const int img = hp / T::HPI, rem = hp % T::HPI;
            const int gy = ty0 + rem / T::HTW - 1, gx = tx0 + rem % T::HTW - 1, ib = img0 + img;
            f32x4 v = {0.f, 0.f, 0.f, 0.f};
            if (((T::HP * 8) % 256 == 0 || q < T::HP * 8) && (unsigned)gy < (unsigned)HS && (unsigned)gx < (unsigned)HS && ib < a.B)
                v = *reinterpret_cast<const f32x4*>(a.in + ((size_t)(ib * HS + gy) * HS + gx) * CIN + ci0 + c4 * 4);
            rin[i] = v;
        }
#pragma unroll
        for (int i = 0; i < 8; ++i) {
            const int q = tid + i * 256;
            const int c4 = q & 7, mm = (q >> 3) & 63, p = q >> 9;
            const int im = mm / (T::TH * T::TW), rem = mm % (T::TH * T::TW);
            const int oy = 2 * (ty0 + rem / T::TW) + (p >> 1), ox = 2 * (tx0 + rem % T::TW) + (p & 1), ib = img0 + im;
            f32x4 v = {0.f, 0.f, 0.f, 0.f};
            if (ib < a.B) v = *reinterpret_cast<const f32x4*>(a.dout + ((size_t)(ib * H + oy) * H + ox) * COUT + n0 + c4 * 4);
            rdo[i] = v;
        }
    };
    if (t0 < t1) fetch(t0);
    for (int mt = t0; mt < t1; ++mt) {
        __syncthreads();
#pragma unroll
        for (int i = 0; i < IQ; ++i) {
            const int q = tid + i * 256;
            if ((T::HP * 8) % 256 == 0 || q < T::HP * 8) *reinterpret_cast<f32x4*>(lds_in + (q >> 3) * CS + (q & 7) * 4) = rin[i];
        }
#pragma unroll
        for (int i = 0; i < 8; ++i) {
            const int q = tid + i * 256;
            *reinterpret_cast<f32x4*>(lds_d + (q >> 9) * 64 * 32 + ((q >> 3) & 63) * 32 + (q & 7) * 4) = rdo[i];
        }
        __syncthreads();
        if (mt + 1 < t1) fetch(mt + 1);
        const float* dph = lds_d + wave * 64 * 32 + li;
#pragma unroll 4
        for (int kk = 0; kk < 32; ++kk) {
            const int mm = 2 * kk + lh;
            const int im = mm / (T::TH * T::TW), rem = mm % (T::TH * T::TW);
            const float* ip = lds_in + ((im * T::HTH + rem / T::TW) * T::HTW + rem % T::TW) * CS + li;
            const float bv = dph[mm * 32];
            bsum += bv;
#pragma unroll
            for (int t = 0; t < 9; ++t)
                acc[t] = __builtin_amdgcn_mfma_f32_32x32x2f32(ip[((t / 3) * T::HTW + t % 3) * CS], bv, acc[t], 0, 0, 0);
        }
    }
    float* out = a.slab + (size_t)split * (36 * CIN * COUT + COUT);
#pragma unroll
    for (int t = 0; t < 9; ++t)
#pragma unroll
        for (int v = 0; v < 16; ++v) {
            const int ci = ci0 + (v & 3) + 8 * (v >> 2) + 4 * lh;
            out[((size_t)(wave * 9 + t) * CIN + ci) * COUT + n0 + li] = acc[t][v];
        }
    __syncthreads();
    bsum += __shfl_xor(bsum, 32, 64);
    if (lh == 0) smem[wave * 32 + li] = bsum;
    __syncthreads();
    if (wave == 0 && lh == 0 && blockIdx.y == 0)
        out[(size_t)36 * CIN * COUT + n0 + li] = (smem[li] + smem[32 + li]) + (smem[64 + li] + smem[96 + li]);
}

struct UpCfg { int cin, cout, hs; };
static UpCfg up_cfg(int layer, int width) {
    return UpCfg{kLayers[layer].cin, kLayers[layer].cout, kLayers[layer].h * (width / 64) / 2};
}
int64_t conv_up_wc_floats(int layer) { return (int64_t)36 * kLayers[layer].cin * kLayers[layer].cout; }

int launch_collapse_w(int layer, const float* w, float* wc, hipStream_t st) {
    const int n = kLayers[layer].cin * kLayers[layer].cout;
    CollapseJobs jobs{{w, nullptr, nullptr}, {wc, nullptr, nullptr}, {n, 0, 0}};
    hipLaunchKernelGGL(collapse_w_kernel, dim3(cdiv(n, 256), 36, 1), dim3(256), 0, st, jobs);
    CVAE_CHECK_LAUNCH();
    return 0;
}
int launch_collapse_w3(const float* const w[3], float* const wc[3], hipStream_t st) {
    CollapseJobs jobs;
    int nmax = 0;
    for (int i = 0; i < 3; ++i) {
        jobs.w[i] = w[i]; jobs.wc[i] = wc[i]; jobs.n[i] = kLayers[5 + i].cin * kLayers[5 + i].cout;
        if (jobs.n[i] > nmax) nmax = jobs.n[i];
    }
    hipLaunchKernelGGL(collapse_w_kernel, dim3(cdiv(nmax, 256), 36, 3), dim3(256), 0, st, jobs);
    CVAE_CHECK_LAUNCH();
    return 0;
}

template <int CIN, int COUT, int HS, int KSPLIT>
static int run_up_fwd(int B, const float* in, const float* wc, const float* bias, float* out, float* ws, hipStream_t st) {
    using T = UpTile<HS>;
    const int64_t slice = (int64_t)B * 4 * HS * HS * COUT;
    UpArgs a{in, wc, bias, nullptr, KSPLIT > 1 ? ws : out, B, slice};
    cvae_probe_begin(st);
    hipLaunchKernelGGL((conv_up_fwd_kernel<CIN, COUT, HS, KSPLIT>), dim3(cdiv(B, T::IMGS) * T::TILES_PER_IMG, COUT / 32, KSPLIT),
                       dim3(256), 0, st, a);
    cvae_probe_end(st);
    CVAE_CHECK_LAUNCH();
    if (KSPLIT > 1) {
        hipLaunchKernelGGL(up_finish_relu_kernel, dim3((unsigned)((slice / 4 + 255) / 256)), dim3(256), 0, st, ws, bias, out,
                           slice / 4, slice, KSPLIT, COUT);
        CVAE_CHECK_LAUNCH();
    }
    return 0;
}

template <int CIN, int COUT, int HS, int NT, int KSPLIT>
static int run_up_dgrad(int B, const float* dout, const float* wc, const float* aux, float* din, float* ws, hipStream_t st) {
    using T = UpTile<HS>;
    const int64_t slice = (int64_t)B * HS * HS * CIN;
    UpArgs a{dout, wc, nullptr, aux, KSPLIT > 1 ? ws : din, B, slice};
    cvae_probe_begin(st);
    hipLaunchKernelGGL((conv_up_dgrad_kernel<CIN, COUT, HS, NT, KSPLIT>), dim3(cdiv(B, T::IMGS) * T::TILES_PER_IMG, CIN / NT, KSPLIT),
                       dim3(256), 0, st, a);
    cvae_probe_end(st);
    CVAE_CHECK_LAUNCH();
    if (KSPLIT > 1) {
        hipLaunchKernelGGL(up_finish_mask_kernel, dim3((unsigned)((slice / 4 + 255) / 256)), dim3(256), 0, st, ws, aux, din,
                           slice / 4, slice, KSPLIT);
        CVAE_CHECK_LAUNCH();
    }
    return 0;
}

static constexpr int UP_KS5 = 4, UP_KS6 = 2;

int64_t conv_up_ws_floats(int layer, int width, int B) {
    const UpCfg c = up_cfg(layer, width);
    const int64_t fwd = (int64_t)B * 4 * c.hs * c.hs * c.cout, dg = (int64_t)B * c.hs * c.hs * c.cin;
    const int ks = layer == 5 ? UP_KS5 : layer == 6 ? UP_KS6 : 0;
    return ks * (fwd > dg ? fwd : dg);
}

int launch_conv_up_fwd(int layer, int width, int B, const float* in, const float* wc, const float* bias, float* out,
                       float* ws, hipStream_t st) {
    if (width == 64) {
        switch (layer) {
            case 5: return run_up_fwd<128, 64, 4, UP_KS5>(B, in, wc, bias, out, ws, st);
            case 6: return run_up_fwd<64, 32, 8, UP_KS6>(B, in, wc, bias, out, ws, st);
            case 7: return run_up_fwd<32, 32, 16, 1>(B, in, wc, bias, out, ws, st);
        }
    }
    if (width == 128) {
        switch (layer) {
            case 5: return run_up_fwd<128, 64, 8, UP_KS5>(B, in, wc, bias, out, ws, st);
            case 6: return run_up_fwd<64, 32, 16, UP_KS6>(B, in, wc, bias, out, ws, st);
            case 7: return run_up_fwd<32, 32, 32, 1>(B, in, wc, bias, out, ws, st);
        }
    }
    cvae_set_error("conv_up_fwd: unsupported layer %d at width %d", layer, width);
    return -2;
}

int launch_conv_up_dgrad(int layer, int width, int B, const float* dout, const float* wc, const float* aux, float* din,
                         float* ws, hipStream_t st) {
    if (width == 64) {
        switch (layer) {
            case 5: return run_up_dgrad<128, 64, 4, 64, UP_KS5>(B, dout, wc, aux, din, ws, st);
            case 6: return run_up_dgrad<64, 32, 8, 64, UP_KS6>(B, dout, wc, aux, din, ws, st);
            case 7: return run_up_dgrad<32, 32, 16, 32, 1>(B, dout, wc, aux, din, ws, st);
        }
    }
    if (width == 128) {
        switch (layer) {
            case 5: return run_up_dgrad<128, 64, 8, 64, UP_KS5>(B, dout, wc, aux, din, ws, st);
            case 6: return run_up_dgrad<64, 32, 16, 64, UP_KS6>(B, dout, wc, aux, din, ws, st);
            case 7: return run_up_dgrad<32, 32, 32, 32, 1>(B, dout, wc, aux, din, ws, st);
        }
    }
    cvae_set_error("conv_up_dgrad: unsupported layer %d at width %d", layer, width);
    return -2;
}

template <int CIN, int COUT, int HS>
static int run_up_wgrad(int B, const float* in, const float* dout, float* dw, float* dbias, float* ws, hipStream_t st,
                        int64_t* need, int bf16_layer = 0, int bf16_width = 64, int* plan = nullptr) {
    using T = UpTile64<HS>;
    const int numTiles = cdiv(B, T::IMGS) * T::TILES_PER_IMG;
    const int bps = (CIN / 32) * (COUT / 32);
    const int cus = cvae_num_cus();
    int Scap = cdiv(2 * cus, bps);
    if (Scap > numTiles) Scap = numTiles;
    int S = cdiv(cus, bps);
    if (S > numTiles) S = numTiles;
    const int tps = cdiv(numTiles, S);
    S = cdiv(numTiles, tps);
    const int64_t nc = (int64_t)36 * CIN * COUT, row = nc + COUT;
    if (plan) return launch_up_wgrad_bf16_main(bf16_layer, bf16_width, B, nullptr, nullptr, nullptr, Scap, &S, st, plan);
    if (need) { *need = (int64_t)(Scap + 17) * row; return 0; }
    if (bf16_layer) {
        int rc = launch_up_wgrad_bf16_main(bf16_layer, bf16_width, B, in, dout, ws, Scap, &S, st);
        if (rc) return rc;
    } else {
        UpWgradArgs a{in, dout, ws, B, numTiles, tps};
        cvae_probe_begin(st);
        hipLaunchKernelGGL((conv_up_wgrad_kernel<CIN, COUT, HS>), dim3(S, CIN / 32, COUT / 32), dim3(256), 0, st, a);
        cvae_probe_end(st);
        CVAE_CHECK_LAUNCH();
    }
    float* mid = ws + (size_t)S * row;
    float* red = mid + (size_t)16 * row;
    { int rc = launch_reduce_slabs(ws, red, row, S, row, st, mid); if (rc) return rc; }
    const float* rows = red;
    const int R = 1;
    static_assert(COUT <= 256, "expand_dw_kernel sums the bias gradient in one workgroup");
    hipLaunchKernelGGL(expand_dw_kernel, dim3(cdiv(CIN * COUT, 256), 25), dim3(256), 0, st, rows, R, row, dw, CIN * COUT, dbias, COUT);
    CVAE_CHECK_LAUNCH();
    return 0;
}

static int dispatch_up_wgrad(int layer, int width, int B, const float* in, const float* dout, float* dw, float* dbias,
                             float* ws, hipStream_t st, int64_t* need, bool bf16 = false, int* plan = nullptr) {
    if (width == 64) {
        switch (layer) {
            case 5: return run_up_wgrad<128, 64, 4>(B, in, dout, dw, dbias, ws, st, need, bf16 ? 5 : 0, 64, plan);
            case 6: return run_up_wgrad<64, 32, 8>(B, in, dout, dw, dbias, ws, st, need, bf16 ? 6 : 0, 64, plan);
            case 7: return run_up_wgrad<32, 32, 16>(B, in, dout, dw, dbias, ws, st, need, bf16 ? 7 : 0, 64, plan);
        }
    }
    if (width == 128) {
        switch (layer) {
            case 5: return run_up_wgrad<128, 64, 8>(B, in, dout, dw, dbias, ws, st, need, bf16 ? 5 : 0, 128, plan);
            case 6: return run_up_wgrad<64, 32, 16>(B, in, dout, dw, dbias, ws, st, need, bf16 ? 6 : 0, 128, plan);
            case 7: return run_up_wgrad<32, 32, 32>(B, in, dout, dw, dbias, ws, st, need, bf16 ? 7 : 0, 128, plan);
        }
    }
    cvae_set_error("conv_up_wgrad: unsupported layer %d at width %d", layer, width);
    return -2;
}
int64_t conv_up_wgrad_ws_floats(int layer, int width, int B) {
    int64_t need = 0;
    if (dispatch_up_wgrad(layer, width, B, nullptr, nullptr, nullptr, nullptr, nullptr, nullptr, &need)) return 0;
    return need;
}
int conv_up_wgrad_bf16_plan(int layer, int width, int B, int plan[3]) {
    return dispatch_up_wgrad(layer, width, B, nullptr, nullptr, nullptr, nullptr, nullptr, nullptr, nullptr, true, plan);
}
int launch_conv_up_wgrad(int layer, int width, int B, const float* in, const float* dout, float* dw, float* dbias,
                         float* ws, hipStream_t st, bool bf16) {
    return dispatch_up_wgrad(layer, width, B, in, dout, dw, dbias, ws, st, nullptr, bf16);
}
```

### critic-vae_amd/lib.py

```python
import ctypes as C
import os
import subprocess

import torch

_HERE = os.path.dirname(os.path.abspath(__file__))
LIB_PATH = os.environ.get("CVAE_LIB") or os.path.join(_HERE, "libcvae_hip.so")
N_SCALARS = 16
SYNC_DOUBLES = 2412
SYNC_POINTS = 9
SCORE_COLS = 8
SCORE_STATE_DOUBLES = 24


class CvaeError(RuntimeError):
    pass


class _Config(C.Structure):
    _fields_ = [("width", C.c_int32), ("max_batch", C.c_int32),
                ("overlap_wgrad", C.c_int32), ("precision", C.c_int32)]


class CrfParams(C.Structure):
    _fields_ = [("w1", C.c_float), ("alpha", C.c_float), ("beta", C.c_float), ("w2", C.c_float),
                ("gamma", C.c_float), ("p_floor", C.c_float), ("iterations", C.c_int32)]


class GuardRecord(C.Structure):
    _fields_ = [("apply", C.c_int32), ("nonfinite", C.c_uint32), ("coef", C.c_float), ("norm", C.c_float),
                ("norm64", C.c_double), ("t", C.c_int64), ("skipped", C.c_int64), ("step_size", C.c_float),
                ("sqrt_bc2", C.c_float), ("gscale", C.c_float), ("beta1", C.c_float), ("beta2", C.c_float),
                ("ticket", C.c_uint32)]


class Objective(C.Structure):
    _fields_ = [("msssim_weight", C.c_float), ("mse_weight", C.c_float), ("kld_weight", C.c_float),
                ("msssim_grad", C.c_int32)]


MSGRAD_REFERENCE, MSGRAD_USED = 0, 1
OPT_MAX_RANGES = 16
OPT_MAX_AUX = 4096


class OptArgs(C.Structure):
    _fields_ = [("decay_mul", C.c_float), ("ema_omd", C.c_float), ("n_ranges", C.c_int32), ("reserved", C.c_int32),
                ("begin", C.c_int64 * OPT_MAX_RANGES), ("end", C.c_int64 * OPT_MAX_RANGES)]


def opt_args(decay_mul=1.0, ema_omd=0.0, ranges=()):
    ranges = list(ranges)
    if len(ranges) > OPT_MAX_RANGES:
        raise ValueError(f"{len(ranges)} decayed ranges: at most {OPT_MAX_RANGES}")
    a = OptArgs(float(decay_mul), float(ema_omd), len(ranges), 0)
    for k, (b, e) in enumerate(ranges):
        a.begin[k], a.end[k] = int(b), int(e)
    return a


TRACE_MAX_SCALARS = 16
TRACE_MAX_TENSORS = 32


class TraceRow(C.Structure):
    _fields_ = [("step", C.c_int64), ("lr", C.c_float), ("applied", C.c_int32), ("nonfinite", C.c_uint32),
                ("grad_norm", C.c_float), ("coef", C.c_float), ("n_scalars", C.c_int32), ("reserved", C.c_uint8 * 32),
                ("scalars", C.c_float * TRACE_MAX_SCALARS)]


class TensorStat(C.Structure):
    _fields_ = [("g2", C.c_double), ("p2", C.c_double), ("u2", C.c_double), ("gmax", C.c_float), ("pmax", C.c_float),
                ("g_nonfinite", C.c_uint32), ("p_nonfinite", C.c_uint32), ("step", C.c_int64)]


def _range_arrays(ranges):
    ranges = [(int(b), int(e)) for b, e in ranges]
    n = len(ranges)
    return n, (C.c_int64 * max(n, 1))(*[b for b, _ in ranges]), (C.c_int64 * max(n, 1))(*[e for _, e in ranges])


def tensor_stats_plan(ranges):
    lib = load()
    n, b, e = _range_arrays(ranges)
    chunk, items, grid = C.c_int32(), C.c_int32(), C.c_int32()
    if lib.cvae_tensor_stats_plan(n, b, e, C.byref(chunk), C.byref(items), C.byref(grid)) != 0:
        raise CvaeError(f"cvae_tensor_stats_plan: {lib.cvae_last_error().decode()}")
    return {"chunk": chunk.value, "items": items.value, "grid": grid.value}


def tensor_stats_scratch_bytes(ranges):
    lib = load()
    n, b, e = _range_arrays(ranges)
    size = lib.cvae_tensor_stats_scratch_bytes(n, b, e)
    if size < 0:
        raise CvaeError(f"cvae_tensor_stats_scratch_bytes: {lib.cvae_last_error().decode()}")
    return size


class AugmentParams(C.Structure):
    _fields_ = [("key", C.c_uint64), ("flip_below", C.c_uint32), ("max_shift", C.c_int32), ("gain_q16", C.c_int32),
                ("reserved", C.c_int32)]


class Panel(C.Structure):
    _fields_ = [("kind", C.c_int32), ("reserved", C.c_int32), ("data", C.c_void_p), ("batch_stride", C.c_int64)]


PANEL_F32_CHW, PANEL_U8_HWC, PANEL_U8_GREY, PANEL_MASK = 0, 1, 2, 3
MAX_PANELS = 8
COMPOSE_CLAMP = 1
CRITIC_KEEP, CRITIC_DECISIONS, CRITIC_TRAIN_FLOATS = 800, 11072, 11876
CRITIC_LOSS = {"bce": 0, "mse": 1}
CRITIC_EMBED_SHAPES = ((8, 32, 32), (8, 16, 16), (8, 8, 8), (16, 4, 4), (32, 1, 1))
CRITIC_IG_MAX_STEPS = 256
CRITIC_OCCLUSION_PATCHES = (4, 8, 16)
CRITIC_SCORE_COLS = 8
CRITIC_SCORE_STATE_DOUBLES = 40


def build(verbose=False):
    r = subprocess.run(["make", "-j8", "-C", os.path.join(_HERE, "csrc")],
                       capture_output=not verbose, text=True)
    if r.returncode != 0:
        raise CvaeError("building libcvae_hip.so failed:\n" + (r.stdout or "") + (r.stderr or ""))
    return LIB_PATH


_lib = None
_p, _i32, _i64, _f = C.c_void_p, C.c_int32, C.c_int64, C.c_float

_SIGS = {
    "cvae_version": (C.c_char_p, []),
    "cvae_last_error": (C.c_char_p, []),
    "cvae_create": (C.c_int, [C.POINTER(_Config), C.POINTER(_p)]),
    "cvae_destroy": (None, [_p]),
    "cvae_param_total": (_i64, [_p]),
    "cvae_param_count": (_i32, [_p]),
    "cvae_param_name": (C.c_char_p, [_p, _i32]),
    "cvae_param_offset": (_i64, [_p, _i32]),
    "cvae_param_numel": (_i64, [_p, _i32]),
    "cvae_workspace_bytes": (_i64, [_p, _i32]),
    "cvae_bn_state_floats": (_i64, [_p]),
    "cvae_ws_offset": (_i64, [_p, _i32, C.c_char_p]),
    "cvae_conv_route": (_i32, [_i32, _i32, _i32, _i32, _i64]),
    "cvae_forward": (C.c_int, [_p, _i32] + [_p] * 9 + [_i32, _p]),
    "cvae_decode": (C.c_int, [_p, _i32] + [_p] * 5),
    "cvae_loss": (C.c_int, [_p, _i32] + [_p] * 10),
    "cvae_loss_obj": (C.c_int, [_p, _i32] + [_p] * 5 + [C.POINTER(Objective)] + [_p] * 5),
    "cvae_backward": (C.c_int, [_p, _i32] + [_p] * 12),
    "cvae_backward_phases": (C.c_int, [_p, _i32] + [_p] * 11 + [_i32, _p]),
    "cvae_grad_bucket": (C.c_int, [_p, _i32, C.POINTER(C.c_int64), C.POINTER(C.c_int64)]),
    "cvae_sync_slot": (C.c_int, [_i32, C.POINTER(C.c_int64), C.POINTER(C.c_int64)]),
    "cvae_forward_stage": (C.c_int, [_p, _i32] + [_p] * 9 + [_i32, _p, _i32, _p]),
    "cvae_loss_stage": (C.c_int, [_p, _i32] + [_p] * 10 + [_i32, _p]),
    "cvae_backward_stage": (C.c_int, [_p, _i32] + [_p] * 12 + [_i32, _p]),
    "cvae_scale_loss_grads": (C.c_int, [_p, _i32] + [_p] * 8),
    "cvae_adam_step": (C.c_int, [_p, _p, _p, _p, _p, _i64, _i32, _f, _f, _f, _f, _f, _p]),
    "cvae_score_cols": (_i32, []),
    "cvae_score_state_bytes": (_i64, []),
    "cvae_score_init": (C.c_int, [_p, _p, _p]),
    "cvae_score": (C.c_int, [_p, _i32] + [_p] * 8),
    "cvae_score_finish": (C.c_int, [_p, _i32, _p, _p, _p]),
    "cvae_guard_state_bytes": (_i64, []),
    "cvae_guard_init": (C.c_int, [_p, _p, _i64, _i64, _p]),
    "cvae_grad_stats": (C.c_int, [_p, _p, _i64, _f, _f, _i32, _f, _f, _f, _p, _p]),
    "cvae_adam_step_guarded": (C.c_int, [_p, _p, _p, _p, _p, _i64, _f, _p, _p]),
    "cvae_adam_step_opt": (C.c_int, [_p, _p, _p, _p, _p, _i64, _i32, _f, _f, _f, _f, _f, C.POINTER(OptArgs), _p, _p, _p, _i32, _p]),
    "cvae_adam_step_guarded_opt": (C.c_int, [_p, _p, _p, _p, _p, _i64, _f, _p, C.POINTER(OptArgs), _p, _p, _p, _i32, _p]),
    "cvae_trace_push": (C.c_int, [_p, _p, _i64, _i64, _f, _p, _i32, _p, _p]),
    "cvae_tensor_stats": (C.c_int, [_p, _p, _p, _p, _p, _i64, _i32, C.POINTER(C.c_int64), C.POINTER(C.c_int64), _i64, _f, _f, _f, _f, _f,
                                    _p, _p, _p, _p]),
    "cvae_tensor_stats_scratch_bytes": (_i64, [_i32, C.POINTER(C.c_int64), C.POINTER(C.c_int64)]),
    "cvae_tensor_stats_plan": (C.c_int, [_i32, C.POINTER(C.c_int64), C.POINTER(C.c_int64)] + [C.POINTER(C.c_int32)] * 3),
    "cvae_grads_to_bf16": (C.c_int, [_p, _p, _p, _i64, _p]),
    "cvae_grads_from_bf16": (C.c_int, [_p, _p, _p, _i64, _p]),
    "cvae_critic_param_count": (_i32, []),
    "cvae_critic_forward": (C.c_int, [_p, _i32, _p, _p, _p, _p]),
    "cvae_critic_train_floats": (_i64, []),
    "cvae_critic_grad_scratch_bytes": (_i64, [_p, _i32]),
    "cvae_critic_grad": (C.c_int, [_p, _i32, _p, _p, _p, _f, _i32] + [_p] * 7),
    "cvae_critic_collect": (C.c_int, [_p, _i32] + [_p] * 9),
    "cvae_critic_saliency": (C.c_int, [_p, _i32, _p, _p, _i32] + [_p] * 6),
    "cvae_critic_occlusion": (C.c_int, [_p, _i32, _p, _p, _i32, _f, _f, _f] + [_p] * 5),
    "cvae_critic_score_state_bytes": (_i64, []),
    "cvae_critic_score_scratch_bytes": (_i64, [_p, _i32]),
    "cvae_critic_score_init": (C.c_int, [_p, _p, _p]),
    "cvae_critic_score": (C.c_int, [_p, _i32, _p, _p, _i64] + [_p] * 6),
    "cvae_preprocess_u8": (C.c_int, [_p, _i32, _p, _p, _p]),
    "cvae_diff_grey": (C.c_int, [_p, _i32, _p, _p, _p, _p]),
    "cvae_curate_select": (C.c_int, [_p, _i32, _p, _i64, _p, _i32, _i64] + [_p] * 6),
    "cvae_gather_frames_u8": (C.c_int, [_p, _i32, _p, _p, _i64, _p, _i64, _p, _p, _p, _i64, _p]),
    "cvae_preprocess_u8_gather": (C.c_int, [_p, _i32, _i32, _p, _p, _i64, _p, _p, _p, _p]),
    "cvae_curate_select_recon": (C.c_int, [_p, _i32, _p, _i64, _p, _i32, _i64] + [_p] * 10),
    "cvae_recon_zcat": (C.c_int, [_p, _i32, _p, _p, _p, _p, _i64, _p, _p]),
    "cvae_gather_f32": (C.c_int, [_p, _i32, _i32, _p, _p, _i64, _p, _p, _p, _p]),
    "cvae_preprocess_u8_gather_aug": (C.c_int, [_p, _i32, _i32, _p, _p, _i64, _p, C.POINTER(AugmentParams), _p, _p, _p, _p]),
    "cvae_gather_f32_aug": (C.c_int, [_p, _i32, _i32, _p, _p, _i64, _p, C.POINTER(AugmentParams), _p, _p, _p, _p]),
    "cvae_diff_normalize": (C.c_int, [_p, _i32, _p, C.c_double, C.c_double, _i32] + [_p] * 6),
    "cvae_mask_counts": (C.c_int, [_p, _i32, _p, _p, _p, _p]),
    "cvae_crf_scratch_bytes": (_i64, [_p, _i32]),
    "cvae_dense_crf": (C.c_int, [_p, _i32, _p, _p, C.POINTER(CrfParams), _p, _p, _p, _p]),
    "cvae_compose_frames": (C.c_int, [_p, _i32, _i32, C.POINTER(Panel), _i32, _i32, _p, _p, _i32, _i32, _i32, _p, _i32, _i32, _p, _p]),
    "cvae_inject_zcat": (C.c_int, [_p, _i32, _i32, _p, _p, _p, _p]),
    "cvae_probe_config": (C.c_int, [_p, C.c_uint32]),
    "cvae_probe_read": (C.c_int, [_p, _i32, C.POINTER(C.c_float), _i32]),
    "cvae_op_scratch_floats": (_i64, [_p, _i32]),
    "cvae_op_bn_partial_floats": (_i64, [_p, _i32, _i32]),
    "cvae_op_msssim_ws_floats": (_i64, [_p, _i32]),
    "cvae_op_conv_fwd": (C.c_int, [_p, _i32, _i32] + [_p] * 7),
    "cvae_op_conv_dgrad": (C.c_int, [_p, _i32, _i32] + [_p] * 6),
    "cvae_op_conv_wgrad": (C.c_int, [_p, _i32, _i32] + [_p] * 6),
    "cvae_op_d4_bwd": (C.c_int, [_p, _i32] + [_p] * 10),
    "cvae_op_bn_pool_act_fwd": (C.c_int, [_p, _i32, _i32] + [_p] * 9 + [_i32, _p]),
    "cvae_op_bn_pool_act_bwd": (C.c_int, [_p, _i32, _i32] + [_p] * 11),
    "cvae_op_conv_tiles_per_partial": (_i32, [_p, _i32, _i32]),
    "cvae_op_conv_wgrad_plan": (C.c_int, [_p, _i32, _i32, C.POINTER(C.c_int32)]),
    "cvae_op_bn_fwd_finalize": (C.c_int, [_p, _i32, _i32, _p, _i32] + [_p] * 6 + [_i32, _p]),
    "cvae_op_msssim": (C.c_int, [_p, _i32] + [_p] * 6),
    "cvae_op_latent_scratch_floats": (_i64, [_p, _i32]),
    "cvae_op_latent_plan": (_i32, [_i32, _i32, _i32, C.POINTER(C.c_int32)]),
    "cvae_op_fc_fwd": (C.c_int, [_p, _i32] + [_p] * 10),
    "cvae_op_decin_fwd": (C.c_int, [_p, _i32] + [_p] * 5),
    "cvae_op_decin_bwd": (C.c_int, [_p, _i32] + [_p] * 8),
    "cvae_op_fc_bwd": (C.c_int, [_p, _i32] + [_p] * 12),
}
EXPORTS = tuple(_SIGS)


def load():
    global _lib
    if _lib is not None:
        return _lib
    if not os.path.exists(LIB_PATH):
        raise CvaeError(f"{LIB_PATH} not found: run __graft_entry__.build() / make -C critic-vae_amd/csrc "
                        "(the HIP library is required; there is no CPU fallback)")
    lib = C.CDLL(LIB_PATH)
    for name, (res, args) in _SIGS.items():
        fn = getattr(lib, name)
        fn.restype, fn.argtypes = res, args
    _lib = lib
    return lib


_DTYPE_NAMES = {torch.float32: "fp32", torch.float64: "fp64", torch.uint8: "uint8", torch.int64: "int64", torch.int32: "int32"}


def _dev_ptr(t, dtype, what):
    if t is None or isinstance(t, int):
        return t
    assert t.is_cuda and t.dtype == dtype and t.is_contiguous(), \
        f"{what}: need a contiguous {_DTYPE_NAMES[dtype]} device tensor, got {t.dtype} {t.device} contiguous={t.is_contiguous()}"
    return t.data_ptr()


def _ptr(t):
    return _dev_ptr(t, torch.float32, "argument")


def _ptr64(t):
    return _dev_ptr(t, torch.float64, "argument")


def sync_slot(point):
    lib = load()
    off, n = C.c_int64(), C.c_int64()
    if lib.cvae_sync_slot(point, C.byref(off), C.byref(n)) != 0:
        raise CvaeError(f"cvae_sync_slot: {lib.cvae_last_error().decode()}")
    return off.value, n.value


LATENT_PLAN_INTS = 15


def latent_plan(width, B, num_cus):
    lib = load()
    out = (C.c_int32 * LATENT_PLAN_INTS)()
    if lib.cvae_op_latent_plan(width, B, num_cus, out) != 0:
        raise CvaeError(f"cvae_op_latent_plan: {lib.cvae_last_error().decode()}")
    v = list(out)
    return {"fc_fwd": {"gemm": v[0]},
            "decin_fwd": {"imgs": v[1], "grid": v[2]},
            "decin_bwd": {"jobs": {"bgemm": (v[3], v[4]), "gemm": (v[5], v[6])}, "grid": v[6]},
            "fc_bwd": {"imgs": v[7], "jobs": {"bgemm": (v[8], v[9]), "dflat": (v[10], v[11]), "colsum": (v[12], v[13])},
                       "grid": v[13], "split": bool(v[14])}}


def _stream():
    return torch.cuda.current_stream().cuda_stream


class Handle:

    PRECISIONS = {"f32": 0, "bf16": 1, "bf16x9": 2, "bf16x6": 3}
    _u8 = staticmethod(lambda t, what: _dev_ptr(t, torch.uint8, what))
    _i32 = staticmethod(lambda t, what: _dev_ptr(t, torch.int32, what))
    _i64 = staticmethod(lambda t, what: _dev_ptr(t, torch.int64, what))

    def __init__(self, width=64, max_batch=256, overlap_wgrad=None, precision="f32"):
        self.lib = load()
        if precision not in self.PRECISIONS:
            raise ValueError(f"precision must be one of {sorted(self.PRECISIONS)}")
        self.precision = precision
        if overlap_wgrad is None:
            overlap_wgrad = os.environ.get("CVAE_OVERLAP_WGRAD") == "1"
        self.overlap_wgrad = bool(overlap_wgrad)
        cfg = _Config(width, max_batch, int(self.overlap_wgrad), self.PRECISIONS[precision])
        h = _p()
        rc = self.lib.cvae_create(C.byref(cfg), C.byref(h))
        self._check(rc)
        self.h = h
        self.width, self.max_batch = width, max_batch
        self.param_total = self.lib.cvae_param_total(h)
        self.layout = {}
        for i in range(self.lib.cvae_param_count(h)):
            self.layout[self.lib.cvae_param_name(h, i).decode()] = (
                self.lib.cvae_param_offset(h, i), self.lib.cvae_param_numel(h, i))
        self.bn_state_floats = self.lib.cvae_bn_state_floats(h)

    def __del__(self):
        try:
            if getattr(self, "h", None):
                self.lib.cvae_destroy(self.h)
                self.h = None
        except Exception:
            pass

    def _check(self, rc):
        if rc != 0:
            raise CvaeError(f"libcvae_hip error {rc}: {self.lib.cvae_last_error().decode()}")

    def workspace_bytes(self, batch):
        return self.lib.cvae_workspace_bytes(self.h, batch)

    def ws_view(self, ws, batch, name, numel):
        off = self.lib.cvae_ws_offset(self.h, batch, name.encode())
        if off < 0:
            raise KeyError(name)
        return ws[off:off + numel]

    def forward(self, B, x, pred, eps, params, bn_state, mu, logvar, recon, ws, train=True):
        self._check(self.lib.cvae_forward(self.h, B, _ptr(x), _ptr(pred), _ptr(eps), _ptr(params), _ptr(bn_state),
                                          _ptr(mu), _ptr(logvar), _ptr(recon), _ptr(ws), int(train), _stream()))

    def decode(self, B, zcat, params, recon, ws):
        self._check(self.lib.cvae_decode(self.h, B, _ptr(zcat), _ptr(params), _ptr(recon), _ptr(ws), _stream()))

    def loss(self, B, x, mu, logvar, recon, ws, scalars, d_recon=None, d_mu=None, d_logvar=None):
        self._check(self.lib.cvae_loss(self.h, B, _ptr(x), _ptr(mu), _ptr(logvar), _ptr(recon), _ptr(ws),
                                       _ptr(scalars), _ptr(d_recon), _ptr(d_mu), _ptr(d_logvar), _stream()))

    def loss_obj(self, B, x, mu, logvar, recon, ws, obj, scalars, d_recon=None, d_mu=None, d_logvar=None):
        if obj is not None and not isinstance(obj, Objective):
            obj = Objective(*obj)
        self._check(self.lib.cvae_loss_obj(self.h, B, _ptr(x), _ptr(mu), _ptr(logvar), _ptr(recon), _ptr(ws),
                                           None if obj is None else C.byref(obj), _ptr(scalars), _ptr(d_recon),
                                           _ptr(d_mu), _ptr(d_logvar), _stream()))

    def backward(self, B, x, pred, eps, params, logvar, recon, d_recon, d_mu, d_logvar, ws, grads, zero_padding=False):
        if zero_padding:
            self._check(self.lib.cvae_backward_phases(self.h, B, _ptr(x), _ptr(pred), _ptr(eps), _ptr(params),
                                                      _ptr(logvar), _ptr(recon), _ptr(d_recon), _ptr(d_mu),
                                                      _ptr(d_logvar), _ptr(ws), _ptr(grads), 15, _stream()))
            return
        self._check(self.lib.cvae_backward(self.h, B, _ptr(x), _ptr(pred), _ptr(eps), _ptr(params), _ptr(logvar),
                                           _ptr(recon), _ptr(d_recon), _ptr(d_mu), _ptr(d_logvar), _ptr(ws),
                                           _ptr(grads), _stream()))

    def scale_loss_grads(self, B, g, d_recon, d_mu, d_logvar, out_recon, out_mu, out_logvar):
        self._check(self.lib.cvae_scale_loss_grads(self.h, B, _ptr(g), _ptr(d_recon), _ptr(d_mu), _ptr(d_logvar),
                                                   _ptr(out_recon), _ptr(out_mu), _ptr(out_logvar), _stream()))

    def grads_to_bf16(self, grads, out_bf16):
        assert out_bf16.is_cuda and out_bf16.dtype == torch.bfloat16 and out_bf16.is_contiguous() and out_bf16.numel() == grads.numel()
        self._check(self.lib.cvae_grads_to_bf16(self.h, _ptr(grads), out_bf16.data_ptr(), grads.numel(), _stream()))

    def grads_from_bf16(self, in_bf16, grads):
        assert in_bf16.is_cuda and in_bf16.dtype == torch.bfloat16 and in_bf16.is_contiguous() and in_bf16.numel() == grads.numel()
        self._check(self.lib.cvae_grads_from_bf16(self.h, in_bf16.data_ptr(), _ptr(grads), grads.numel(), _stream()))

    def backward_phase(self, phase, B, x, pred, eps, params, logvar, recon, d_recon, d_mu, d_logvar, ws, grads):
        self._check(self.lib.cvae_backward_phases(self.h, B, _ptr(x), _ptr(pred), _ptr(eps), _ptr(params), _ptr(logvar),
                                                  _ptr(recon), _ptr(d_recon), _ptr(d_mu), _ptr(d_logvar), _ptr(ws),
                                                  _ptr(grads), 1 << phase, _stream()))

    def grad_bucket(self, phase):
        off, n = C.c_int64(), C.c_int64()
        self._check(self.lib.cvae_grad_bucket(self.h, phase, C.byref(off), C.byref(n)))
        return off.value, n.value

    sync_slot = staticmethod(sync_slot)

    def forward_stage(self, stage, B, x, pred, eps, params, bn_state, mu, logvar, recon, ws, sync, train=True):
        self._check(self.lib.cvae_forward_stage(self.h, B, _ptr(x), _ptr(pred), _ptr(eps), _ptr(params), _ptr(bn_state),
                                                _ptr(mu), _ptr(logvar), _ptr(recon), _ptr(ws), int(train), _ptr64(sync),
                                                stage, _stream()))

    def loss_stage(self, stage, B, x, mu, logvar, recon, ws, scalars, d_recon, d_mu, d_logvar, sync):
        self._check(self.lib.cvae_loss_stage(self.h, B, _ptr(x), _ptr(mu), _ptr(logvar), _ptr(recon), _ptr(ws),
                                             _ptr(scalars), _ptr(d_recon), _ptr(d_mu), _ptr(d_logvar), _ptr64(sync),
                                             stage, _stream()))

    def backward_stage(self, stage, B, x, pred, eps, params, logvar, recon, d_recon, d_mu, d_logvar, ws, grads, sync):
        self._check(self.lib.cvae_backward_stage(self.h, B, _ptr(x), _ptr(pred), _ptr(eps), _ptr(params), _ptr(logvar),
                                                 _ptr(recon), _ptr(d_recon), _ptr(d_mu), _ptr(d_logvar), _ptr(ws),
                                                 _ptr(grads), _ptr64(sync), stage, _stream()))

    def adam_step(self, params, grads, m, v, step, lr, b1=0.9, b2=0.999, eps=1e-8, grad_scale=1.0):
        self._check(self.lib.cvae_adam_step(self.h, _ptr(params), _ptr(grads), _ptr(m), _ptr(v), params.numel(),
                                            step, lr, b1, b2, eps, grad_scale, _stream()))

    def score_cols(self):
        return self.lib.cvae_score_cols()

    def score_state_bytes(self):
        return self.lib.cvae_score_state_bytes()

    def score_state(self, device):
        state = torch.empty(self.lib.cvae_score_state_bytes() // 8, dtype=torch.float64, device=device)
        self.score_init(state)
        return state

    def _score_ptr(self, state):
        if state is None:
            return None
        ptr = _ptr64(state)
        assert isinstance(state, int) or state.numel() * 8 >= self.lib.cvae_score_state_bytes(), "score state: too small"
        return ptr

    def score_init(self, state):
        self._check(self.lib.cvae_score_init(self.h, self._score_ptr(state), _stream()))

    def score(self, B, x, mu, logvar, recon, ws, per_image=None, state=None):
        self._check(self.lib.cvae_score(self.h, B, _ptr(x), _ptr(mu), _ptr(logvar), _ptr(recon), _ptr(ws), _ptr(per_image),
                                        self._score_ptr(state), _stream()))

    def score_finish(self, state, scalars, width=None):
        self._check(self.lib.cvae_score_finish(self.h, self.width if width is None else width, self._score_ptr(state),
                                               _ptr(scalars), _stream()))

    def guard_state(self, device, applied=0, skipped=0):
        state = torch.empty((self.lib.cvae_guard_state_bytes() + 7) // 8, dtype=torch.int64, device=device)
        self.guard_init(state, applied, skipped)
        return state

    def guard_init(self, state, applied=0, skipped=0):
        self._check(self.lib.cvae_guard_init(self.h, self._guard_ptr(state), int(applied), int(skipped), _stream()))

# ... 353 lines not shown
```

### include/cvae.h

```cpp
#ifndef CVAE_H
#define CVAE_H

#include <stddef.h>
#include <stdint.h>

#ifdef __cplusplus
extern "C" {
#endif

typedef struct cvae_handle_s* cvae_handle;

typedef struct cvae_config {
    int32_t width;
    int32_t max_batch;
    int32_t overlap_wgrad;
    int32_t precision;
} cvae_config;

enum { CVAE_OK = 0, CVAE_EINVAL = -1, CVAE_EUNSUPPORTED = -2, CVAE_ENOWS = -3 };

#define CVAE_N_SCALARS 16

const char* cvae_version(void);
const char* cvae_last_error(void);

int  cvae_create(const cvae_config* cfg, cvae_handle* out);
void cvae_destroy(cvae_handle h);

int64_t     cvae_param_total(cvae_handle h);
int32_t     cvae_param_count(cvae_handle h);
const char* cvae_param_name(cvae_handle h, int32_t i);
int64_t     cvae_param_offset(cvae_handle h, int32_t i);
int64_t     cvae_param_numel(cvae_handle h, int32_t i);

int64_t cvae_workspace_bytes(cvae_handle h, int32_t batch);

int64_t cvae_bn_state_floats(cvae_handle h);

int cvae_forward(cvae_handle h, int32_t batch, const float* x, const float* pred, const float* eps,
                 const float* params, float* bn_state, float* mu, float* logvar, float* recon,
                 void* ws, int32_t train, void* stream);

int cvae_decode(cvae_handle h, int32_t batch, const float* zcat, const float* params, float* recon,
                void* ws, void* stream);

int cvae_loss(cvae_handle h, int32_t batch, const float* x, const float* mu, const float* logvar,
              const float* recon, void* ws, float* scalars, float* d_recon, float* d_mu,
              float* d_logvar, void* stream);

typedef struct cvae_objective {
    float   msssim_weight;
    float   mse_weight;
    float   kld_weight;
    int32_t msssim_grad;
} cvae_objective;
enum { CVAE_MSGRAD_REFERENCE = 0, CVAE_MSGRAD_USED = 1 };
int cvae_loss_obj(cvae_handle h, int32_t batch, const float* x, const float* mu, const float* logvar,
                  const float* recon, void* ws, const cvae_objective* obj, float* scalars, float* d_recon,
                  float* d_mu, float* d_logvar, void* stream);

#define CVAE_SCORE_COLS 8
#define CVAE_SCORE_STATE_DOUBLES 24
int32_t cvae_score_cols(void);
int64_t cvae_score_state_bytes(void);
int cvae_score_init(cvae_handle h, void* state, void* stream);
int cvae_score(cvae_handle h, int32_t batch, const float* x, const float* mu, const float* logvar, const float* recon,
               void* ws, float* per_image_or_null, void* state_or_null, void* stream);
int cvae_score_finish(cvae_handle h, int32_t width, void* state, float* scalars, void* stream);

int cvae_backward(cvae_handle h, int32_t batch, const float* x, const float* pred, const float* eps,
                  const float* params, const float* logvar, const float* recon, const float* d_recon,
                  const float* d_mu, const float* d_logvar, void* ws, float* grads, void* stream);

int cvae_backward_phases(cvae_handle h, int32_t batch, const float* x, const float* pred, const float* eps,
                         const float* params, const float* logvar, const float* recon, const float* d_recon,
                         const float* d_mu, const float* d_logvar, void* ws, float* grads, int32_t phase_mask,
                         void* stream);
int cvae_grad_bucket(cvae_handle h, int32_t phase, int64_t* offset, int64_t* numel);

#define CVAE_SYNC_DOUBLES 2412
int cvae_sync_slot(int32_t point, int64_t* offset, int64_t* count);
int cvae_forward_stage(cvae_handle h, int32_t batch, const float* x, const float* pred, const float* eps,
                       const float* params, float* bn_state, float* mu, float* logvar, float* recon, void* ws,
                       int32_t train, double* sync, int32_t stage, void* stream);
int cvae_loss_stage(cvae_handle h, int32_t batch, const float* x, const float* mu, const float* logvar,
                    const float* recon, void* ws, float* scalars, float* d_recon, float* d_mu, float* d_logvar,
                    double* sync, int32_t stage, void* stream);
int cvae_backward_stage(cvae_handle h, int32_t batch, const float* x, const float* pred, const float* eps,
                        const float* params, const float* logvar, const float* recon, const float* d_recon,
                        const float* d_mu, const float* d_logvar, void* ws, float* grads, double* sync, int32_t stage,
                        void* stream);

int cvae_scale_loss_grads(cvae_handle h, int32_t batch, const float* gscale, const float* d_recon,
                          const float* d_mu, const float* d_logvar, float* d_recon_out, float* d_mu_out,
                          float* d_logvar_out, void* stream);

int cvae_grads_to_bf16(cvae_handle h, const float* grads, void* out_bf16, int64_t n, void* stream);
int cvae_grads_from_bf16(cvae_handle h, const void* in_bf16, float* grads, int64_t n, void* stream);

int cvae_adam_step(cvae_handle h, float* params, const float* grads, float* exp_avg,
                   float* exp_avg_sq, int64_t n, int32_t step, float lr, float beta1, float beta2,
                   float eps, float grad_scale, void* stream);

typedef struct cvae_guard_record {
    int32_t  apply;
    uint32_t nonfinite;
    float    coef;
    float    norm;
    double   norm64;
    int64_t  t;
    int64_t  skipped;
    float    step_size;
    float    sqrt_bc2;
    float    gscale;
    float    beta1, beta2;
    uint32_t ticket;
} cvae_guard_record;
int64_t cvae_guard_state_bytes(void);
int cvae_guard_init(cvae_handle h, void* state, int64_t applied, int64_t skipped, void* stream);
int cvae_grad_stats(cvae_handle h, const float* grads, int64_t n, float grad_scale, float max_norm, int32_t skip_nonfinite,
                    float lr, float beta1, float beta2, void* state, void* stream);
int cvae_adam_step_guarded(cvae_handle h, float* params, const float* grads, float* exp_avg, float* exp_avg_sq, int64_t n,
                           float eps, const void* state, void* stream);

#define CVAE_OPT_MAX_RANGES 16
typedef struct cvae_opt_args {
    float   decay_mul;
    float   ema_omd;
    int32_t n_ranges;
    int32_t reserved;
    int64_t begin[CVAE_OPT_MAX_RANGES], end[CVAE_OPT_MAX_RANGES];
} cvae_opt_args;
int cvae_adam_step_opt(cvae_handle h, float* params, const float* grads, float* exp_avg, float* exp_avg_sq, int64_t n,
                       int32_t step, float lr, float beta1, float beta2, float eps, float grad_scale,
                       const cvae_opt_args* opt , float* ema ,
                       float* aux, float* aux_ema, int32_t n_aux , void* stream);
int cvae_adam_step_guarded_opt(cvae_handle h, float* params, const float* grads, float* exp_avg, float* exp_avg_sq, int64_t n,
                               float eps, const void* state, const cvae_opt_args* opt, float* ema, float* aux, float* aux_ema,
                               int32_t n_aux, void* stream);

#define CVAE_TRACE_MAX_SCALARS 16
typedef struct cvae_trace_row {
    int64_t  step;
    float    lr;
    int32_t  applied;
    uint32_t nonfinite;
    float    grad_norm, coef;
    int32_t  n_scalars;
    uint8_t  reserved[32];
    float    scalars[16];
} cvae_trace_row;
int cvae_trace_push(cvae_handle h, void* ring, int64_t capacity, int64_t step, float lr,
                    const float* loss_scalars, int32_t n_scalars, const void* guard_state_or_null, void* stream);

#define CVAE_TRACE_MAX_TENSORS 32
typedef struct cvae_tensor_stat {
    double   g2, p2, u2;
    float    gmax, pmax;
    uint32_t g_nonfinite, p_nonfinite;
    int64_t  step;
} cvae_tensor_stat;
int cvae_tensor_stats(cvae_handle h, const float* params, const float* grads, const float* exp_avg, const float* exp_avg_sq,
                      int64_t n, int32_t n_tensors, const int64_t* begin, const int64_t* end ,
                      int64_t step, float lr, float beta1, float beta2, float eps, float grad_scale,
                      const void* guard_state_or_null, cvae_tensor_stat* out, void* scratch, void* stream);
int64_t cvae_tensor_stats_scratch_bytes(int32_t n_tensors, const int64_t* begin, const int64_t* end);
int cvae_tensor_stats_plan(int32_t n_tensors, const int64_t* begin, const int64_t* end,
                           int32_t* chunk, int32_t* items, int32_t* grid);

int32_t cvae_critic_param_count(void);
int cvae_critic_forward(cvae_handle h, int32_t batch, const float* x, const float* critic_params,
                        float* pred, void* stream);

#define CVAE_CRITIC_KEEP      800
#define CVAE_CRITIC_DECISIONS 11072
enum { CVAE_CRITIC_LOSS_BCE = 0, CVAE_CRITIC_LOSS_MSE = 1 };
int64_t cvae_critic_train_floats(void);
int64_t cvae_critic_grad_scratch_bytes(cvae_handle h, int32_t batch);
int cvae_critic_grad(cvae_handle h, int32_t batch, const float* x, const float* target, const uint8_t* keep_or_null,
                     float dropout_p, int32_t loss_kind, const float* critic_params, float* grads, float* pred,
                     float* loss_scalars, uint8_t* decisions_or_null, void* scratch, void* stream);

#define CVAE_CRITIC_SCORE_COLS 8
#define CVAE_CRITIC_SCORE_STATE_DOUBLES 40
int64_t cvae_critic_score_state_bytes(void);
int64_t cvae_critic_score_scratch_bytes(cvae_handle h, int32_t batch);
int cvae_critic_score_init(cvae_handle h, void* state, void* stream);
int cvae_critic_score(cvae_handle h, int32_t batch, const uint8_t* frames_hwc, const float* targets, int64_t n_frames,
                      const int64_t* idx_or_null, const float* critic_params, float* per_frame_or_null,
                      void* state_or_null, void* scratch, void* stream);

#define CVAE_CRITIC_IG_MAX_STEPS 256
int cvae_critic_collect(cvae_handle h, int32_t batch, const float* x, const float* critic_params, float* pred,
                        float* e1_or_null, float* e2_or_null, float* e3_or_null, float* e4_or_null, float* e5_or_null,
                        void* stream);
int cvae_critic_saliency(cvae_handle h, int32_t batch, const float* x, const float* critic_params, int32_t steps,
                         float* pred, float* grad_or_null, float* map, float* max_values, uint8_t* decisions_or_null,
                         void* stream);
int cvae_critic_occlusion(cvae_handle h, int32_t batch, const float* x, const float* critic_params, int32_t patch,
                          float fill_r, float fill_g, float fill_b, float* pred, float* drop, float* map,
                          float* max_values, void* stream);

int cvae_preprocess_u8(cvae_handle h, int32_t batch, const uint8_t* frames_hwc, float* x, void* stream);


int cvae_curate_select(cvae_handle h, int32_t n_traj, const int64_t* traj_offsets, int64_t n_frames,
                       const float* preds, int32_t collect, int64_t total_images, int64_t* running,
                       int64_t* counts, int64_t* first, int64_t* span, int64_t* sel, void* stream);

int cvae_gather_frames_u8(cvae_handle h, int32_t width, const uint8_t* src_frames, const float* src_preds_or_null,
                          int64_t n_src, const int64_t* sel, int64_t max_count, const int64_t* span,
                          uint8_t* dst_frames, float* dst_preds_or_null, int64_t capacity, void* stream);

int cvae_preprocess_u8_gather(cvae_handle h, int32_t batch, int32_t width, const uint8_t* frames_hwc,
                              const float* preds, int64_t n_frames, const int64_t* idx, float* x,
                              float* pred, void* stream);


int cvae_curate_select_recon(cvae_handle h, int32_t n_traj, const int64_t* traj_offsets, int64_t n_frames,
                             const float* preds, int32_t collect, int64_t total_images, int64_t* running,
                             int64_t* counts, int64_t* first, int64_t* sel_first, int64_t* span, int64_t* ent_frame,
                             int32_t* ent_kind, int64_t* ent_sel, int64_t* sel, void* stream);

int cvae_recon_zcat(cvae_handle h, int32_t n_entries, const int64_t* ent_sel, const int32_t* ent_kind, const float* mu,
                    const float* sel_preds, int64_t n_sel, float* zcat, void* stream);

int cvae_gather_f32(cvae_handle h, int32_t batch, int32_t width, const float* frames, const float* preds,
                    int64_t n_frames, const int64_t* idx, float* x, float* pred, void* stream);

typedef struct cvae_augment {
    uint64_t key;
    uint32_t flip_below;
    int32_t  max_shift;
    int32_t  gain_q16;
    int32_t  reserved;
} cvae_augment;
int cvae_preprocess_u8_gather_aug(cvae_handle h, int32_t batch, int32_t width, const uint8_t* frames_hwc,
                                  const float* preds, int64_t n_frames, const int64_t* idx, const cvae_augment* aug,
                                  float* x, float* pred, int32_t* applied_or_null, void* stream);
int cvae_gather_f32_aug(cvae_handle h, int32_t batch, int32_t width, const float* frames, const float* preds,
                        int64_t n_frames, const int64_t* idx, const cvae_augment* aug, float* x, float* pred,
                        int32_t* applied_or_null, void* stream);

int cvae_diff_grey(cvae_handle h, int32_t batch, const float* recon_one, const float* recon_zero,
                   float* diff, void* stream);


int cvae_diff_normalize(cvae_handle h, int32_t batch, const float* diff, double mean_max, double diff_factor,
                        int32_t thr, const uint8_t* gt_or_null, uint8_t* diff_u8, uint8_t* mask_or_null,
                        int64_t* frame_counts_or_null, int64_t* hist_or_null, void* stream);

int cvae_mask_counts(cvae_handle h, int32_t batch, const uint8_t* mask, const uint8_t* gt,
                     int64_t* frame_counts, void* stream);

typedef struct cvae_crf_params {
    float w1, alpha, beta, w2, gamma, p_floor;
    int32_t iterations;
} cvae_crf_params;
int64_t cvae_crf_scratch_bytes(cvae_handle h, int32_t batch);
int cvae_dense_crf(cvae_handle h, int32_t batch, const uint8_t* frames_hwc, const float* prob1,
                   const cvae_crf_params* params, uint8_t* labels, float* q1_or_null, void* scratch,
                   void* stream);


enum { CVAE_PANEL_F32_CHW = 0, CVAE_PANEL_U8_HWC = 1, CVAE_PANEL_U8_GREY = 2, CVAE_PANEL_MASK = 3 };
#define CVAE_MAX_PANELS 8
#define CVAE_COMPOSE_CLAMP 1
typedef struct cvae_panel {
    int32_t kind;
    int32_t reserved;
    const void* data;
    int64_t batch_stride;
} cvae_panel;

int cvae_compose_frames(cvae_handle h, int32_t batch, int32_t n_panels, const cvae_panel* panels, int32_t row_offset,
                        int32_t flags, const uint8_t* overlay_or_null, const uint8_t* atlas_or_null, int32_t n_labels,
                        int32_t label_h, int32_t label_w, const int32_t* label_idx, int32_t label_x, int32_t label_y,
                        uint8_t* out, void* stream);

int cvae_inject_zcat(cvae_handle h, int32_t n_images, int32_t n_rewards, const float* mu, const float* rewards,
                     float* zcat, void* stream);

int64_t cvae_ws_offset(cvae_handle h, int32_t batch, const char* name);

int32_t cvae_conv_route(int32_t precision, int32_t width, int32_t layer, int32_t dgrad, int64_t batch);

int cvae_probe_config(cvae_handle h, uint32_t mask);
int cvae_probe_read(cvae_handle h, int32_t id, float* ms_host, int32_t cap);

int64_t cvae_op_scratch_floats(cvae_handle h, int32_t batch);
int64_t cvae_op_bn_partial_floats(cvae_handle h, int32_t layer, int32_t batch);
int64_t cvae_op_msssim_ws_floats(cvae_handle h, int32_t batch);

int cvae_op_conv_fwd(cvae_handle h, int32_t layer, int32_t batch, const float* in, const float* w,
                     const float* bias, float* out, float* bn_partials, void* scratch, void* stream);
int cvae_op_conv_dgrad(cvae_handle h, int32_t layer, int32_t batch, const float* dout,
                       const float* w, const float* mask_src, float* din, void* scratch, void* stream);
int cvae_op_conv_wgrad(cvae_handle h, int32_t layer, int32_t batch, const float* in,
                       const float* dout, float* dw, float* dbias, void* scratch, void* stream);
int cvae_op_d4_bwd(cvae_handle h, int32_t batch, const float* o3, const float* d_recon,
                   const float* recon, const float* w, float* dout, float* d_o3, float* dw,
                   float* db, void* scratch, void* stream);
int cvae_op_bn_pool_act_fwd(cvae_handle h, int32_t layer, int32_t batch, const float* y,
                            const float* bn_partials, const float* gamma, const float* beta,
                            float* run_mean, float* run_var, float* coef, float* a, void* scratch,
                            int32_t train, void* stream);
int32_t cvae_op_conv_tiles_per_partial(cvae_handle h, int32_t layer, int32_t batch);
int cvae_op_conv_wgrad_plan(cvae_handle h, int32_t layer, int32_t batch, int32_t* out);
int cvae_op_bn_fwd_finalize(cvae_handle h, int32_t layer, int32_t batch, const float* bn_partials,
                            int32_t tiles_per_partial, const float* gamma, const float* beta,
                            float* run_mean, float* run_var, float* coef, void* scratch,
                            int32_t train, void* stream);
int cvae_op_bn_pool_act_bwd(cvae_handle h, int32_t layer, int32_t batch, const float* y,
                            const float* a, const float* da, const float* coef, const float* gamma,
                            float* dy, float* dgamma, float* dbeta, float* dbias, void* scratch,
                            void* stream);
int cvae_op_msssim(cvae_handle h, int32_t batch, const float* img1, const float* img2, void* ws,
                   float* scalars, float* d_img1, void* stream);

int64_t cvae_op_latent_scratch_floats(cvae_handle h, int32_t batch);
#define CVAE_LATENT_PLAN_INTS 15
int32_t cvae_op_latent_plan(int32_t width, int32_t batch, int32_t num_cus, int32_t* out);
int cvae_op_fc_fwd(cvae_handle h, int32_t batch, const float* flat, const float* wfc, const float* bfc,
                   const float* eps, const float* pred, float* mu, float* logvar, float* zcat,
                   void* scratch, void* stream);
int cvae_op_decin_fwd(cvae_handle h, int32_t batch, const float* zcat, const float* wd, const float* bd,
                      float* h_out, void* stream);
int cvae_op_decin_bwd(cvae_handle h, int32_t batch, const float* zcat, const float* dh, const float* wd,
                      float* dwd, float* dbd, float* dzcat, void* scratch, void* stream);
int cvae_op_fc_bwd(cvae_handle h, int32_t batch, const float* flat, const float* wfc, const float* dzcat,
                   const float* eps, const float* logvar, const float* dmu_loss, const float* dlv_loss,
                   float* dwfc, float* dbfc, float* dflat, void* scratch, void* stream);

#ifdef __cplusplus
}
#endif
#endif
```

Measured before the change: 89980.

## Add optional 8-wave decoder conv kernels and pipeline row4x4 tap loads

Adds an 8-wave (512-thread) variant of the decoder 4x4 row and upsample conv kernels that splits output channel blocks across two wave halves. It is chosen by a planner that is currently hard-disabled unless an env var forces it, and a query API is added to report the choice. Separately, the 4x4 row kernel's inner tap loop becomes a templated helper that double-buffers LDS operand loads into registers and interleaves them with MFMAs using scheduling barriers. This is meant to hide LDS latency, at the cost of extra register pressure.

```diff
diff --git a/critic-vae_amd/csrc/api.hip b/critic-vae_amd/csrc/api.hip
--- a/critic-vae_amd/csrc/api.hip
+++ b/critic-vae_amd/csrc/api.hip
@@ -59,6 +59,17 @@
     if ((width != 64 && width != 128) || layer < 0 || layer > 3 || precision < 0 || precision > 3 || batch < 1 || batch > 0x7fffffffLL) return CVAE_EINVAL;
     if (layer == 0 && (precision != 1 || dgrad != 0)) return CVAE_EINVAL;
     return conv_route(precision, layer, width, dgrad != 0, batch).family;
+}
+extern "C" int32_t cvae_dec_conv_waves(int32_t width, int32_t layer, int32_t dgrad, int64_t batch, int32_t cus) {
+    if ((width != 64 && width != 128) || layer < 4 || layer > 7 || batch < 1 || batch > 0x7fffffffLL || cus < 1) return CVAE_EINVAL;
+    DecWavesPlan plan{cus, 0};
+    const int B = (int)batch;
+    int rc;
+    if (layer == 4) rc = dgrad ? launch_conv_dgrad(4, width, B, nullptr, nullptr, nullptr, nullptr, nullptr, nullptr, &plan)
+                               : launch_conv_fwd(4, width, B, nullptr, nullptr, nullptr, nullptr, nullptr, nullptr, nullptr, &plan);
+    else rc = dgrad ? launch_conv_up_dgrad(layer, width, B, nullptr, nullptr, nullptr, nullptr, nullptr, nullptr, &plan)
+                    : launch_conv_up_fwd(layer, width, B, nullptr, nullptr, nullptr, nullptr, nullptr, nullptr, &plan);
+    return rc ? CVAE_EINVAL : plan.waves;
 }
 
 struct ParamEntry { std::string name; int64_t offset, numel; };
diff --git a/critic-vae_amd/csrc/common.h b/critic-vae_amd/csrc/common.h
--- a/critic-vae_amd/csrc/common.h
+++ b/critic-vae_amd/csrc/common.h
@@ -163,11 +163,14 @@
 };
 ConvRoute conv_route(int precision, int layer, int width, bool dgrad, int64_t B);
 
+int dec_conv_waves(int64_t workgroups, int cus = 0);
+struct DecWavesPlan { int cus, waves; };
+
 int launch_conv_fwd(int layer, int width, int B, const float* in, const float* w, const float* bias,
-                    float* out, float* bnpart, float* ws, hipStream_t st);
+                    float* out, float* bnpart, float* ws, hipStream_t st, DecWavesPlan* plan = nullptr);
 int64_t conv_fwd_ws_floats(int layer, int width, int B);
 int launch_conv_dgrad(int layer, int width, int B, const float* dout, const float* w,
-                      const float* mask_src, float* din, float* ws, hipStream_t st);
+                      const float* mask_src, float* din, float* ws, hipStream_t st, DecWavesPlan* plan = nullptr);
 int64_t conv_dgrad_ws_floats(int layer, int width, int B);
 bool conv_bf16_supported(int layer, int width);
 int64_t conv_bf16_pack_floats(int ns);
@@ -231,9 +234,9 @@
 int launch_collapse_w3(const float* const w[3], float* const wc[3], hipStream_t st);
 int64_t conv_up_ws_floats(int layer, int width, int B);
 int launch_conv_up_fwd(int layer, int width, int B, const float* in, const float* wc, const float* bias,
-                       float* out, float* ws, hipStream_t st);
+                       float* out, float* ws, hipStream_t st, DecWavesPlan* plan = nullptr);
 int launch_conv_up_dgrad(int layer, int width, int B, const float* dout, const float* wc, const float* aux,
-                         float* din, float* ws, hipStream_t st);
+                         float* din, float* ws, hipStream_t st, DecWavesPlan* plan = nullptr);
 int64_t conv_up_wgrad_ws_floats(int layer, int width, int B);
 int launch_conv_up_wgrad(int layer, int width, int B, const float* in, const float* dout, float* dw,
                          float* dbias, float* ws, hipStream_t st, bool bf16 = false);
diff --git a/critic-vae_amd/csrc/conv_mfma.hip b/critic-vae_amd/csrc/conv_mfma.hip
--- a/critic-vae_amd/csrc/conv_mfma.hip
+++ b/critic-vae_amd/csrc/conv_mfma.hip
@@ -222,9 +222,34 @@
     return 0;
 }
 
-template <int KCH, int NCH, bool DGRAD, int NT, int KSPLIT>
-__global__ __launch_bounds__(256) void conv4x4_row_kernel(ConvArgs a) {
-    constexpr int NB = NT / 32;
+template <int NTAP, int NB, bool DGRAD, int NT, int KC, int KCP, int PS, int AS, int BS>
+__device__ __forceinline__ void row4x4_taps(f32x16 (&acc)[NB], const float* as, const float* bs) {
+    constexpr int NK = NTAP * (KC / 2);
+    float af[2], bf[2][NB];
+    auto ld = [&](int i, int b) {
+        const int s = i / (KC / 2), j = i % (KC / 2);
+        af[b] = as[s * AS + (2 * j) * PS];
+#pragma unroll
+        for (int nb = 0; nb < NB; ++nb) bf[b][nb] = DGRAD ? bs[s * BS + nb * 32 * KCP + 2 * j] : bs[s * BS + (2 * j) * NT + nb * 32];
+    };
+    ld(0, 0);
+    __builtin_amdgcn_sched_group_barrier(0x100, 1 + NB, 0);
+#pragma unroll
+    for (int i = 0; i < NK; ++i) {
+        if (i + 1 < NK) ld(i + 1, (i + 1) & 1);
+#pragma unroll
+        for (int nb = 0; nb < NB; ++nb) acc[nb] = __builtin_amdgcn_mfma_f32_32x32x2f32(af[i & 1], bf[i & 1][nb], acc[nb], 0, 0, 0);
+        __builtin_amdgcn_sched_group_barrier(0x008, 1, 0);
+        if (i + 1 < NK) __builtin_amdgcn_sched_group_barrier(0x100, 1 + NB, 0);
+        if (NB > 1) __builtin_amdgcn_sched_group_barrier(0x008, NB - 1, 0);
+        __builtin_amdgcn_sched_barrier(0);
+    }
+}
+
+template <int KCH, int NCH, bool DGRAD, int NT, int KSPLIT, int WAVES = 4>
+__global__ __launch_bounds__(WAVES * 64, WAVES == 8 && !DGRAD ? 4 : WAVES / 4) void conv4x4_row_kernel(ConvArgs a) {
+    static_assert(WAVES == 4 || (WAVES == 8 && NT == 64), "four waves, or two halves of four with one channel block each");
+    constexpr int NB = NT / 32 / (WAVES / 4), NTH = WAVES * 64;
     constexpr int KC = KChunk<NT>::KC, KCP = KChunk<NT>::KCP, QPP = KC / 4;
     constexpr int PXS = 33, PS = 16 * PXS + 2;
     constexpr int IN_FLOATS = KC * PS;
@@ -233,11 +258,13 @@
     float* lds_in = smem;
     float* lds_w = smem + IN_FLOATS;
     static_assert(IN_FLOATS % 4 == 0, "weight slab stays 16-byte aligned");
-    const int tid = threadIdx.x, lane = tid & 63, wave = tid >> 6, li = lane & 31, lh = lane >> 5;
+    const int tid = threadIdx.x, lane = tid & 63, li = lane & 31, lh = lane >> 5;
+    const int wave = WAVES == 8 ? (tid >> 6) & 3 : tid >> 6;
+    const int nb0 = WAVES == 8 ? tid >> 8 : 0;
     const int ya = (blockIdx.x & 1) * 2, img0 = (blockIdx.x >> 1) * 32, n0 = blockIdx.y * NT;
     const int r0 = ya == 0 ? 1 : 0, r1 = ya == 0 ? 4 : 3;
     const int aBase = lh * PS + li;
-    const int bBase = DGRAD ? (li * KCP + lh) : (lh * NT + li);
+    const int bBase = DGRAD ? ((nb0 * 32 + li) * KCP + lh) : (lh * NT + nb0 * 32 + li);
 
     f32x16 acc[2][NB];
 #pragma unroll
@@ -247,13 +274,13 @@
 #pragma unroll
             for (int v = 0; v < 16; ++v) acc[t][nb][v] = 0.f;
 
-    constexpr int WQ = 5 * KC * NT / 4, WPT = (WQ + 255) / 256;
+    constexpr int WQ = 5 * KC * NT / 4, WPT = (WQ + NTH - 1) / NTH;
     f32x4 wreg[WPT];
     auto load_w = [&](int cc, int r) {
 #pragma unroll
         for (int i = 0; i < WPT; ++i) {
-            const int q = tid + i * 256;
-            if (WQ % 256 == 0 || q < WQ) {
+            const int q = tid + i * NTH;
+            if (WQ % NTH == 0 || q < WQ) {
                 const float* src;
                 if (!DGRAD) {
                     const int row = q / (NT / 4), c4 = q % (NT / 4);
@@ -271,8 +298,8 @@
     auto store_w = [&]() {
 #pragma unroll
         for (int i = 0; i < WPT; ++i) {
-            const int q = tid + i * 256;
-            if (WQ % 256 == 0 || q < WQ) {
+            const int q = tid + i * NTH;
+            if (WQ % NTH == 0 || q < WQ) {
                 if (!DGRAD) {
                     *reinterpret_cast<f32x4*>(lds_w + q * 4) = wreg[i];
                 } else {
@@ -283,12 +310,12 @@
             }
         }
     };
-    constexpr int NQ = 512 * QPP, IPT = NQ / 256;
+    constexpr int NQ = 512 * QPP, IPT = NQ / NTH;
     f32x4 ireg[IPT];
     auto load_input = [&](int cc) {
 #pragma unroll
         for (int i = 0; i < IPT; ++i) {
-            const int q = tid + i * 256, c4 = q % QPP, hp = q / QPP, ib = img0 + (hp >> 4);
+            const int q = tid + i * NTH, c4 = q % QPP, hp = q / QPP, ib = img0 + (hp >> 4);
             f32x4 v = {0.f, 0.f, 0.f, 0.f};
             if (ib < a.B) v = *reinterpret_cast<const f32x4*>(a.in + ((size_t)ib * 16 + (hp & 15)) * KCH + cc * KC + c4 * 4);
             ireg[i] = v;
@@ -297,7 +324,7 @@
     auto store_input = [&]() {
 #pragma unroll
         for (int i = 0; i < IPT; ++i) {
-            const int q = tid + i * 256, c4 = q % QPP, hp = q / QPP;
+            const int q = tid + i * NTH, c4 = q % QPP, hp = q / QPP;
             float* d = lds_in + (c4 * 4) * PS + (hp & 15) * PXS + (hp >> 4);
             d[0] = ireg[i].x; d[PS] = ireg[i].y; d[2 * PS] = ireg[i].z; d[3 * PS] = ireg[i].w;
         }
@@ -323,20 +350,12 @@
                 if ((unsigned)yi > 3u) continue;
                 const int xc = wave ^ t;
                 const int s0 = xc < 2 ? 2 - xc : 0, s1 = xc > 1 ? 5 - xc : 4;
-                const float* ap = lds_in + aBase + (yi * 4 + xc - 2) * PXS;
-                for (int s = s0; s <= s1; ++s) {
-                    const float* as = ap + s * PXS;
-                    const float* bs = lds_w + bBase + (DGRAD ? s * NT * KCP : s * KC * NT);
-#pragma unroll
-                    for (int j = 0; j < KC / 2; ++j) {
-                        const float av = as[(2 * j) * PS];
-#pragma unroll
-                        for (int nb = 0; nb < NB; ++nb) {
-                            const float bv = DGRAD ? bs[nb * 32 * KCP + 2 * j] : bs[(2 * j) * NT + nb * 32];
-                            acc[t][nb] = __builtin_amdgcn_mfma_f32_32x32x2f32(av, bv, acc[t][nb], 0, 0, 0);
-                        }
-                    }
-                }
+                constexpr int BS = DGRAD ? NT * KCP : KC * NT;
+                const float* as = lds_in + aBase + (yi * 4 + xc - 2 + s0) * PXS;
+                const float* bs = lds_w + bBase + s0 * BS;
+                const bool four = s1 - s0 == 3;
+                if (four) row4x4_taps<4, NB, DGRAD, NT, KC, KCP, PS, PXS, BS>(acc[t], as, bs);
+                if (!four) row4x4_taps<3, NB, DGRAD, NT, KC, KCP, PS, PXS, BS>(acc[t], as, bs);
             }
         }
     vm_drained();
@@ -348,15 +367,28 @@
 #pragma unroll
             for (int v = 0; v < 16; ++v) {
                 const int ib = img0 + (v & 3) + 8 * (v >> 2) + 4 * lh;
-                if (ib < a.B) out[((size_t)ib * 16 + (ya + t) * 4 + (wave ^ t)) * NCH + n0 + nb * 32 + li] = acc[t][nb][v];
-            }
+                if (ib < a.B) out[((size_t)ib * 16 + (ya + t) * 4 + (wave ^ t)) * NCH + n0 + (nb0 + nb) * 32 + li] = acc[t][nb][v];
+            }
+}
+
+int dec_conv_waves(int64_t workgroups, int cus) {
+    static const int forced = [] { const char* e = getenv("CVAE_DEC_WAVES"); const int n = e ? atoi(e) : 0; return n == 4 || n == 8 ? n : 0; }();
+    if (forced) return forced;
+    constexpr bool kEightWaveRoute = false;
+    if (!kEightWaveRoute) return 4;
+    if (cus <= 0) cus = cvae_num_cus();
+    return workgroups <= cus ? 8 : 4;
 }
 
 template <int KCH, int NCH, bool DGRAD, int NT, int KSPLIT>
-static int run4x4(const ConvArgs& a, hipStream_t st) {
+static int run4x4(const ConvArgs& a, hipStream_t st, DecWavesPlan* plan) {
     static_assert(KCH % KChunk<NT>::KC == 0 && NCH % NT == 0, "channel tiling");
+    const dim3 grid(cdiv(a.B, 32) * 2, NCH / NT, KSPLIT);
+    const int waves = dec_conv_waves((int64_t)grid.x * grid.y * grid.z, plan ? plan->cus : 0);
+    if (plan) { plan->waves = waves; return 0; }
     cvae_probe_begin(st);
-    hipLaunchKernelGGL((conv4x4_row_kernel<KCH, NCH, DGRAD, NT, KSPLIT>), dim3(cdiv(a.B, 32) * 2, NCH / NT, KSPLIT), dim3(256), 0, st, a);
+    if (waves == 8) hipLaunchKernelGGL((conv4x4_row_kernel<KCH, NCH, DGRAD, NT, KSPLIT, 8>), grid, dim3(512), 0, st, a);
+    else hipLaunchKernelGGL((conv4x4_row_kernel<KCH, NCH, DGRAD, NT, KSPLIT>), grid, dim3(256), 0, st, a);
     cvae_probe_end(st);
     CVAE_CHECK_LAUNCH();
     return 0;
@@ -395,7 +427,8 @@
 int launch_conv_mfma_ps(int layer, int width, bool dgrad, int B, const float* in, const float* w, const float* bias, float* out, float* bnpart, hipStream_t st);
 
 int launch_conv_fwd(int layer, int width, int B, const float* in, const float* w, const float* bias,
-                    float* out, float* bnpart, float* ws, hipStream_t st) {
+                    float* out, float* bnpart, float* ws, hipStream_t st, DecWavesPlan* plan) {
+    if (plan && !(layer == 4 && width == 64)) { plan->waves = 4; return 0; }
     if (conv_route(0, layer, width, false, B).family == CONV_PS) return launch_conv_mfma_ps(layer, width, false, B, in, w, bias, out, bnpart, st);
     ConvArgs a{in, w, bias, nullptr, out, bnpart, B, 0};
     if (width == 64) {
@@ -406,8 +439,8 @@
             case 4: {
                 const int64_t slice = (int64_t)B * 4 * 4 * 128;
                 a.out = ws; a.sliceFloats = slice;
-                int rc = run4x4<256, 128, false, 64, D0_KSPLIT>(a, st);
-                if (rc) return rc;
+                int rc = run4x4<256, 128, false, 64, D0_KSPLIT>(a, st, plan);
+                if (rc || plan) return rc;
                 hipLaunchKernelGGL(splitk_bias_relu_kernel<float>, dim3((unsigned)((slice / 4 + 255) / 256)), dim3(256), 0, st,
                                    ws, bias, out, slice / 4, slice, D0_KSPLIT, 128);
                 CVAE_CHECK_LAUNCH();
@@ -434,14 +467,15 @@
 }
 
 int launch_conv_dgrad(int layer, int width, int B, const float* dout, const float* w,
-                      const float* mask_src, float* din, float* ws, hipStream_t st) {
+                      const float* mask_src, float* din, float* ws, hipStream_t st, DecWavesPlan* plan) {
+    if (plan && !(layer == 4 && width == 64)) { plan->waves = 4; return 0; }
     if (!mask_src && conv_route(0, layer, width, true, B).family == CONV_PS) return launch_conv_mfma_ps(layer, width, true, B, dout, w, nullptr, din, nullptr, st);
     ConvArgs a{dout, w, nullptr, mask_src, din, nullptr, B, 0};
-    if (width == 64 && layer == 4 && ws != nullptr) {
+    if (width == 64 && layer == 4 && (ws != nullptr || plan)) {
         const int64_t slice = (int64_t)B * 16 * 256;
         a.out = ws; a.sliceFloats = slice;
-        int rc = run4x4<128, 256, true, 64, D0_DGRAD_KSPLIT>(a, st);
-        if (rc) return rc;
+        int rc = run4x4<128, 256, true, 64, D0_DGRAD_KSPLIT>(a, st, plan);
+        if (rc || plan) return rc;
         return launch_reduce_slabs(ws, din, slice, D0_DGRAD_KSPLIT, slice, st, nullptr);
     }
     if (width == 64) {
diff --git a/critic-vae_amd/csrc/conv_up.hip b/critic-vae_amd/csrc/conv_up.hip
--- a/critic-vae_amd/csrc/conv_up.hip
+++ b/critic-vae_amd/csrc/conv_up.hip
@@ -62,36 +62,40 @@
     int64_t sliceFloats;
 };
 
-template <int CIN, int COUT, int HS, int KSPLIT>
-__global__ __launch_bounds__(256) void conv_up_fwd_kernel(UpArgs a) {
+template <int CIN, int COUT, int HS, int KSPLIT, int WAVES = 4>
+__global__ __launch_bounds__(WAVES * 64, WAVES == 8 ? 4 : 1) void conv_up_fwd_kernel(UpArgs a) {
     using T = UpTile<HS>;
-    constexpr int NT = 32, H = 2 * HS;
+    static_assert(WAVES == 4 || WAVES == 8, "four waves, or two halves of four");
+    constexpr int NT = 32, H = 2 * HS, NTH = WAVES * 64, PH = 16 / WAVES;
     constexpr int IN_FLOATS = KC * T::PS, W_FLOATS = 12 * KC * NT;
     __shared__ __attribute__((aligned(16))) float smem[IN_FLOATS + W_FLOATS];
     float* lds_in = smem;
     float* lds_w = smem + IN_FLOATS;
-    const int tid = threadIdx.x, lane = tid & 63, wave = tid >> 6, li = lane & 31, lh = lane >> 5;
+    const int tid = threadIdx.x, lane = tid & 63, li = lane & 31, lh = lane >> 5;
+    const int wave = WAVES == 8 ? (tid >> 6) & 3 : tid >> 6;
+    const int p0 = WAVES == 8 ? (tid >> 8) * PH : 0;
     const int mt = xcd_tile(blockIdx.x, gridDim.x), n0 = blockIdx.y * NT;
     const int tileInImg = mt % T::TILES_PER_IMG, img0 = (mt / T::TILES_PER_IMG) * T::IMGS;
     const int ty0 = (tileInImg / T::TILES_X) * T::TH, tx0 = (tileInImg % T::TILES_X) * T::TW;
     const int m = wave * 32 + li;
     const int pimg = m / (T::TH * T::TW), prem = m % (T::TH * T::TW);
     const int aBase = lh * T::PS + pimg * T::HPI + (prem / T::TW) * T::HTW + (prem % T::TW);
-    const int bBase = lh * NT + li;
-
-    f32x16 acc[4];
-#pragma unroll
-    for (int p = 0; p < 4; ++p)
+    const int bBase = lh * NT + li + p0 * 3 * KC * NT;
+
+    f32x16 acc[PH];
+#pragma unroll
+    for (int p = 0; p < PH; ++p)
 #pragma unroll
         for (int v = 0; v < 16; ++v) acc[p][v] = 0.f;
 
-    constexpr int WQ = 12 * KC * NT / 4, WPT = WQ / 256;
+    constexpr int WQ = 12 * KC * NT / 4, WPT = WQ / NTH;
+    static_assert(WQ % NTH == 0, "whole float4 units per thread");
     f32x4 wreg[WPT];
     auto load_w = [&](int st) {
         const int cc = st / 3, ar = st % 3;
 #pragma unroll
         for (int i = 0; i < WPT; ++i) {
-            const int q = tid + i * 256;
+            const int q = tid + i * NTH;
             const int row = q / (NT / 4), c4 = q % (NT / 4);
             const int pb = row / KC, kc = row % KC, p = pb / 3, b = pb % 3;
             wreg[i] = *reinterpret_cast<const f32x4*>(
@@ -100,19 +104,19 @@
     };
     auto store_w = [&]() {
 #pragma unroll
-        for (int i = 0; i < WPT; ++i) *reinterpret_cast<f32x4*>(lds_w + (tid + i * 256) * 4) = wreg[i];
-    };
-    constexpr int NQ = T::HP * (KC / 4), IPT = (NQ + 255) / 256;
+        for (int i = 0; i < WPT; ++i) *reinterpret_cast<f32x4*>(lds_w + (tid + i * NTH) * 4) = wreg[i];
+    };
+    constexpr int NQ = T::HP * (KC / 4), IPT = (NQ + NTH - 1) / NTH;
     f32x4 ireg[IPT];
     auto load_input = [&](int cc) {
 #pragma unroll
         for (int i = 0; i < IPT; ++i) {
-            const int q = tid + i * 256;
+            const int q = tid + i * NTH;
             const int c4 = q & 3, hp = q >> 2;
             const int img = hp / T::HPI, rem = hp - img * T::HPI;
             const int gy = ty0 + rem / T::HTW - 1, gx = tx0 + rem % T::HTW - 1, ib = img0 + img;
             f32x4 v = {0.f, 0.f, 0.f, 0.f};
-            if ((NQ % 256 == 0 || q < NQ) && (unsigned)gy < (unsigned)HS && (unsigned)gx < (unsigned)HS && ib < a.B)
+            if ((NQ % NTH == 0 || q < NQ) && (unsigned)gy < (unsigned)HS && (unsigned)gx < (unsigned)HS && ib < a.B)
                 v = *reinterpret_cast<const f32x4*>(a.in + ((size_t)(ib * HS + gy) * HS + gx) * CIN + cc * KC + c4 * 4);
             ireg[i] = v;
         }
@@ -120,8 +124,8 @@
     auto store_input = [&]() {
 #pragma unroll
         for (int i = 0; i < IPT; ++i) {
-            const int q = tid + i * 256;
-            if (NQ % 256 == 0 || q < NQ) {
+            const int q = tid + i * NTH;
+            if (NQ % NTH == 0 || q < NQ) {
                 float* d = lds_in + ((q & 3) * 4) * T::PS + (q >> 2);
                 d[0] = ireg[i].x; d[T::PS] = ireg[i].y; d[2 * T::PS] = ireg[i].z; d[3 * T::PS] = ireg[i].w;
             }
@@ -150,41 +154,45 @@
             for (int j = 0; j < KC / 2; ++j) {
                 const float av = ap[(2 * j) * T::PS + b];
 #pragma unroll
-                for (int p = 0; p < 4; ++p)
+                for (int p = 0; p < PH; ++p)
                     acc[p] = __builtin_amdgcn_mfma_f32_32x32x2f32(av, lds_w[bBase + ((p * 3 + b) * KC + 2 * j) * NT], acc[p], 0, 0, 0);
             }
     }
     vm_drained();
     float* out = KSPLIT > 1 ? a.out + (size_t)blockIdx.z * a.sliceFloats : a.out;
 #pragma unroll
-    for (int p = 0; p < 4; ++p)
+    for (int pl = 0; pl < PH; ++pl)
 #pragma unroll
         for (int v = 0; v < 16; ++v) {
+            const int p = p0 + pl;
             const int mm = wave * 32 + (v & 3) + 8 * (v >> 2) + 4 * lh;
             const int im = mm / (T::TH * T::TW), rem = mm % (T::TH * T::TW);
             const int oy = 2 * (ty0 + rem / T::TW) + (p >> 1), ox = 2 * (tx0 + rem % T::TW) + (p & 1), ib = img0 + im;
-            float x = acc[p][v] + bv;
+            float x = acc[pl][v] + bv;
             if (KSPLIT == 1) x = fmaxf(x, 0.f);
             if (ib < a.B) out[((size_t)(ib * H + oy) * H + ox) * COUT + n0 + li] = x;
         }
 }
 
-template <int CIN, int COUT, int HS, int NT, int KSPLIT>
-__global__ __launch_bounds__(256) void conv_up_dgrad_kernel(UpArgs a) {
+template <int CIN, int COUT, int HS, int NT, int KSPLIT, int WAVES = 4>
+__global__ __launch_bounds__(WAVES * 64, WAVES == 8 ? 4 : 1) void conv_up_dgrad_kernel(UpArgs a) {
     using T = UpTile<HS>;
-    constexpr int NB = NT / 32, H = 2 * HS;
+    static_assert(WAVES == 4 || (WAVES == 8 && NT == 64), "four waves, or two halves of four with one channel block each");
+    constexpr int NB = NT / 32 / (WAVES / 4), H = 2 * HS, NTH = WAVES * 64;
     constexpr int IN_FLOATS = KC * T::PS, W_FLOATS = 9 * NT * KCP;
     __shared__ __attribute__((aligned(16))) float smem[IN_FLOATS + W_FLOATS];
     float* lds_in = smem;
     float* lds_w = smem + IN_FLOATS;
-    const int tid = threadIdx.x, lane = tid & 63, wave = tid >> 6, li = lane & 31, lh = lane >> 5;
+    const int tid = threadIdx.x, lane = tid & 63, li = lane & 31, lh = lane >> 5;
+    const int wave = WAVES == 8 ? (tid >> 6) & 3 : tid >> 6;
+    const int nb0 = WAVES == 8 ? tid >> 8 : 0;
     const int mt = xcd_tile(blockIdx.x, gridDim.x), n0 = blockIdx.y * NT;
     const int tileInImg = mt % T::TILES_PER_IMG, img0 = (mt / T::TILES_PER_IMG) * T::IMGS;
     const int ty0 = (tileInImg / T::TILES_X) * T::TH, tx0 = (tileInImg % T::TILES_X) * T::TW;
     const int m = wave * 32 + li;
     const int pimg = m / (T::TH * T::TW), prem = m % (T::TH * T::TW);
     const int aBase = lh * T::PS + pimg * T::HPI + (prem / T::TW + 2) * T::HTW + (prem % T::TW) + 2;
-    const int bBase = li * KCP + lh;
+    const int bBase = (nb0 * 32 + li) * KCP + lh;
 
     f32x16 acc[NB];
 #pragma unroll
@@ -192,14 +200,14 @@
 #pragma unroll
         for (int v = 0; v < 16; ++v) acc[nb][v] = 0.f;
 
-    constexpr int WQ = 9 * NT * KC / 4, WPT = (WQ + 255) / 256;
+    constexpr int WQ = 9 * NT * KC / 4, WPT = (WQ + NTH - 1) / NTH;
     f32x4 wreg[WPT];
     auto load_w = [&](int st) {
         const int cc = st / 4, p = st % 4;
 #pragma unroll
         for (int i = 0; i < WPT; ++i) {
-            const int q = tid + i * 256;
-            if (WQ % 256 == 0 || q < WQ) {
+            const int q = tid + i * NTH;
+            if (WQ % NTH == 0 || q < WQ) {
                 const int c4 = q & 3, rown = q >> 2, n = rown % NT, t = rown / NT;
                 wreg[i] = *reinterpret_cast<const f32x4*>(
                     a.wc + ((size_t)(p * 9 + t) * CIN + n0 + n) * COUT + cc * KC + c4 * 4);
@@ -209,25 +217,25 @@
     auto store_w = [&]() {
 #pragma unroll
         for (int i = 0; i < WPT; ++i) {
-            const int q = tid + i * 256;
-            if (WQ % 256 == 0 || q < WQ) {
+            const int q = tid + i * NTH;
+            if (WQ % NTH == 0 || q < WQ) {
                 float* d = lds_w + (q >> 2) * KCP + (q & 3) * 4;
                 d[0] = wreg[i].x; d[1] = wreg[i].y; d[2] = wreg[i].z; d[3] = wreg[i].w;
             }
         }
     };
-    constexpr int NQ = T::HP * (KC / 4), IPT = (NQ + 255) / 256;
+    constexpr int NQ = T::HP * (KC / 4), IPT = (NQ + NTH - 1) / NTH;
     f32x4 ireg[IPT];
     auto load_input = [&](int st) {
         const int cc = st / 4, py = (st % 4) >> 1, px = st & 1;
 #pragma unroll
         for (int i = 0; i < IPT; ++i) {
-            const int q = tid + i * 256;
+            const int q = tid + i * NTH;
             const int c4 = q & 3, hp = q >> 2;
             const int img = hp / T::HPI, rem = hp - img * T::HPI;
             const int yy = ty0 + rem / T::HTW - 1, xx = tx0 + rem % T::HTW - 1, ib = img0 + img;
             f32x4 v = {0.f, 0.f, 0.f, 0.f};
-            if ((NQ % 256 == 0 || q < NQ) && (unsigned)yy < (unsigned)HS && (unsigned)xx < (unsigned)HS && ib < a.B)
+            if ((NQ % NTH == 0 || q < NQ) && (unsigned)yy < (unsigned)HS && (unsigned)xx < (unsigned)HS && ib < a.B)
                 v = *reinterpret_cast<const f32x4*>(
                     a.in + ((size_t)(ib * H + 2 * yy + py) * H + 2 * xx + px) * COUT + cc * KC + c4 * 4);
             ireg[i] = v;
@@ -236,8 +244,8 @@
     auto store_input = [&]() {
 #pragma unroll
         for (int i = 0; i < IPT; ++i) {
-            const int q = tid + i * 256;
-            if (NQ % 256 == 0 || q < NQ) {
+            const int q = tid + i * NTH;
+            if (NQ % NTH == 0 || q < NQ) {
                 float* d = lds_in + ((q & 3) * 4) * T::PS + (q >> 2);
                 d[0] = ireg[i].x; d[T::PS] = ireg[i].y; d[2 * T::PS] = ireg[i].z; d[3 * T::PS] = ireg[i].w;
             }
@@ -276,7 +284,7 @@
         for (int v = 0; v < 16; ++v) {
             const int mm = wave * 32 + (v & 3) + 8 * (v >> 2) + 4 * lh;
             const int im = mm / (T::TH * T::TW), rem = mm % (T::TH * T::TW), ib = img0 + im;
-            o[nb][v] = ((size_t)(ib * HS + ty0 + rem / T::TW) * HS + tx0 + rem % T::TW) * CIN + n0 + nb * 32 + li;
+            o[nb][v] = ((size_t)(ib * HS + ty0 + rem / T::TW) * HS + tx0 + rem % T::TW) * CIN + n0 + (nb0 + nb) * 32 + li;
             if (KSPLIT == 1) mk[nb][v] = a.aux[ib < a.B ? o[nb][v] : 0];
         }
 #pragma unroll
@@ -447,14 +455,21 @@
     return 0;
 }
 
-template <int CIN, int COUT, int HS, int KSPLIT>
-static int run_up_fwd(int B, const float* in, const float* wc, const float* bias, float* out, float* ws, hipStream_t st) {
+template <int CIN, int COUT, int HS, int KSPLIT, bool W8 = false>
+static int run_up_fwd(int B, const float* in, const float* wc, const float* bias, float* out, float* ws, hipStream_t st, DecWavesPlan* plan) {
     using T = UpTile<HS>;
     const int64_t slice = (int64_t)B * 4 * HS * HS * COUT;
+    const dim3 grid(cdiv(B, T::IMGS) * T::TILES_PER_IMG, COUT / 32, KSPLIT);
+    const int waves = W8 ? dec_conv_waves((int64_t)grid.x * grid.y * grid.z, plan ? plan->cus : 0) : 4;
+    if (plan) { plan->waves = waves; return 0; }
     UpArgs a{in, wc, bias, nullptr, KSPLIT > 1 ? ws : out, B, slice};
     cvae_probe_begin(st);
-    hipLaunchKernelGGL((conv_up_fwd_kernel<CIN, COUT, HS, KSPLIT>), dim3(cdiv(B, T::IMGS) * T::TILES_PER_IMG, COUT / 32, KSPLIT),
-                       dim3(256), 0, st, a);
+    if constexpr (W8) {
+        if (waves == 8) hipLaunchKernelGGL((conv_up_fwd_kernel<CIN, COUT, HS, KSPLIT, 8>), grid, dim3(512), 0, st, a);
+        else hipLaunchKernelGGL((conv_up_fwd_kernel<CIN, COUT, HS, KSPLIT>), grid, dim3(256), 0, st, a);
+    } else {
+        hipLaunchKernelGGL((conv_up_fwd_kernel<CIN, COUT, HS, KSPLIT>), grid, dim3(256), 0, st, a);
+    }
     cvae_probe_end(st);
     CVAE_CHECK_LAUNCH();
     if (KSPLIT > 1) {
@@ -465,14 +480,21 @@
     return 0;
 }
 
-template <int CIN, int COUT, int HS, int NT, int KSPLIT>
-static int run_up_dgrad(int B, const float* dout, const float* wc, const float* aux, float* din, float* ws, hipStream_t st) {
+template <int CIN, int COUT, int HS, int NT, int KSPLIT, bool W8 = false>
+static int run_up_dgrad(int B, const float* dout, const float* wc, const float* aux, float* din, float* ws, hipStream_t st, DecWavesPlan* plan) {
     using T = UpTile<HS>;
     const int64_t slice = (int64_t)B * HS * HS * CIN;
+    const dim3 grid(cdiv(B, T::IMGS) * T::TILES_PER_IMG, CIN / NT, KSPLIT);
+    const int waves = W8 ? dec_conv_waves((int64_t)grid.x * grid.y * grid.z, plan ? plan->cus : 0) : 4;
+    if (plan) { plan->waves = waves; return 0; }
     UpArgs a{dout, wc, nullptr, aux, KSPLIT > 1 ? ws : din, B, slice};
     cvae_probe_begin(st);
-    hipLaunchKernelGGL((conv_up_dgrad_kernel<CIN, COUT, HS, NT, KSPLIT>), dim3(cdiv(B, T::IMGS) * T::TILES_PER_IMG, CIN / NT, KSPLIT),
-                       dim3(256), 0, st, a);
+    if constexpr (W8) {
+        if (waves == 8) hipLaunchKernelGGL((conv_up_dgrad_kernel<CIN, COUT, HS, NT, KSPLIT, 8>), grid, dim3(512), 0, st, a);
+        else hipLaunchKernelGGL((conv_up_dgrad_kernel<CIN, COUT, HS, NT, KSPLIT>), grid, dim3(256), 0, st, a);
+    } else {
+        hipLaunchKernelGGL((conv_up_dgrad_kernel<CIN, COUT, HS, NT, KSPLIT>), grid, dim3(256), 0, st, a);
+    }
     cvae_probe_end(st);
     CVAE_CHECK_LAUNCH();
     if (KSPLIT > 1) {
@@ -493,19 +515,19 @@
 }
 
 int launch_conv_up_fwd(int layer, int width, int B, const float* in, const float* wc, const float* bias, float* out,
-                       float* ws, hipStream_t st) {
+                       float* ws, hipStream_t st, DecWavesPlan* plan) {
     if (width == 64) {
         switch (layer) {
-            case 5: return run_up_fwd<128, 64, 4, UP_KS5>(B, in, wc, bias, out, ws, st);
-            case 6: return run_up_fwd<64, 32, 8, UP_KS6>(B, in, wc, bias, out, ws, st);
-            case 7: return run_up_fwd<32, 32, 16, 1>(B, in, wc, bias, out, ws, st);
+            case 5: return run_up_fwd<128, 64, 4, UP_KS5, true>(B, in, wc, bias, out, ws, st, plan);
+            case 6: return run_up_fwd<64, 32, 8, UP_KS6, true>(B, in, wc, bias, out, ws, st, plan);
+            case 7: return run_up_fwd<32, 32, 16, 1>(B, in, wc, bias, out, ws, st, plan);
         }
     }
     if (width == 128) {
         switch (layer) {
-            case 5: return run_up_fwd<128, 64, 8, UP_KS5>(B, in, wc, bias, out, ws, st);
-            case 6: return run_up_fwd<64, 32, 16, UP_KS6>(B, in, wc, bias, out, ws, st);
-            case 7: return run_up_fwd<32, 32, 32, 1>(B, in, wc, bias, out, ws, st);
+            case 5: return run_up_fwd<128, 64, 8, UP_KS5>(B, in, wc, bias, out, ws, st, plan);
+            case 6: return run_up_fwd<64, 32, 16, UP_KS6>(B, in, wc, bias, out, ws, st, plan);
+            case 7: return run_up_fwd<32, 32, 32, 1>(B, in, wc, bias, out, ws, st, plan);
         }
     }
     cvae_set_error("conv_up_fwd: unsupported layer %d at width %d", layer, width);
@@ -513,19 +535,19 @@
 }
 
 int launch_conv_up_dgrad(int layer, int width, int B, const float* dout, const float* wc, const float* aux, float* din,
-                         float* ws, hipStream_t st) {
+                         float* ws, hipStream_t st, DecWavesPlan* plan) {
     if (width == 64) {
         switch (layer) {
-            case 5: return run_up_dgrad<128, 64, 4, 64, UP_KS5>(B, dout, wc, aux, din, ws, st);
-            case 6: return run_up_dgrad<64, 32, 8, 64, UP_KS6>(B, dout, wc, aux, din, ws, st);
-            case 7: return run_up_dgrad<32, 32, 16, 32, 1>(B, dout, wc, aux, din, ws, st);
+            case 5: return run_up_dgrad<128, 64, 4, 64, UP_KS5, true>(B, dout, wc, aux, din, ws, st, plan);
+            case 6: return run_up_dgrad<64, 32, 8, 64, UP_KS6, true>(B, dout, wc, aux, din, ws, st, plan);
+            case 7: return run_up_dgrad<32, 32, 16, 32, 1>(B, dout, wc, aux, din, ws, st, plan);
         }
     }
     if (width == 128) {
         switch (layer) {
-            case 5: return run_up_dgrad<128, 64, 8, 64, UP_KS5>(B, dout, wc, aux, din, ws, st);
-            case 6: return run_up_dgrad<64, 32, 16, 64, UP_KS6>(B, dout, wc, aux, din, ws, st);
-            case 7: return run_up_dgrad<32, 32, 32, 32, 1>(B, dout, wc, aux, din, ws, st);
+            case 5: return run_up_dgrad<128, 64, 8, 64, UP_KS5>(B, dout, wc, aux, din, ws, st, plan);
+            case 6: return run_up_dgrad<64, 32, 16, 64, UP_KS6>(B, dout, wc, aux, din, ws, st, plan);
+            case 7: return run_up_dgrad<32, 32, 32, 32, 1>(B, dout, wc, aux, din, ws, st, plan);
         }
     }
     cvae_set_error("conv_up_dgrad: unsupported layer %d at width %d", layer, width);
diff --git a/critic-vae_amd/lib.py b/critic-vae_amd/lib.py
--- a/critic-vae_amd/lib.py
+++ b/critic-vae_amd/lib.py
@@ -144,6 +144,7 @@
     "cvae_bn_state_floats": (_i64, [_p]),
     "cvae_ws_offset": (_i64, [_p, _i32, C.c_char_p]),
     "cvae_conv_route": (_i32, [_i32, _i32, _i32, _i32, _i64]),
+    "cvae_dec_conv_waves": (_i32, [_i32, _i32, _i32, _i64, _i32]),
     "cvae_forward": (C.c_int, [_p, _i32] + [_p] * 9 + [_i32, _p]),
     "cvae_decode": (C.c_int, [_p, _i32] + [_p] * 5),
     "cvae_loss": (C.c_int, [_p, _i32] + [_p] * 10),
diff --git a/include/cvae.h b/include/cvae.h
--- a/include/cvae.h
+++ b/include/cvae.h
@@ -284,6 +284,8 @@
 int64_t cvae_ws_offset(cvae_handle h, int32_t batch, const char* name);
 
 int32_t cvae_conv_route(int32_t precision, int32_t width, int32_t layer, int32_t dgrad, int64_t batch);
+
+int32_t cvae_dec_conv_waves(int32_t width, int32_t layer, int32_t dgrad, int64_t batch, int32_t cus);
 
 int cvae_probe_config(cvae_handle h, uint32_t mask);
 int cvae_probe_read(cvae_handle h, int32_t id, float* ms_host, int32_t cap);
```

Result: no change. 89980 (-0.0%).
